# cfpark00/vdm4cdm

Hardware: AMD Instinct MI355X
Metric: 3D voxels/sec UNet fwd+bwd @128^3 (VDM training step) (higher is better)
Workload: dtype bf16; 1 GPU; c3: 128^3 conditional VDM (trainVDM3D128_c_c thick_lowbatch), chs [32, 64, 128, 256], batch 2/GPU, full training step (diffuse + UNet fwd + ELBO + UNet bwd + clip + AdamW), dropout 0.1; global_batch=2, cube=128, parallelism=dp1

## Files before the change

include/vdm4cdm_hip.h:

```cpp
#ifndef VDM4CDM_HIP_H
#define VDM4CDM_HIP_H

#include <stddef.h>
#include <stdint.h>

#ifdef __cplusplus
extern "C" {
#endif

#define VDM_ABI_VERSION 15

typedef enum { VDM_OK = 0, VDM_ERR_ARG = -1, VDM_ERR_HIP = -2, VDM_ERR_UNSUPPORTED = -3 } vdm_status;
typedef enum { VDM_F32 = 0, VDM_BF16 = 1 } vdm_dtype;
typedef enum { VDM_PAD_ZEROS = 0, VDM_PAD_CIRCULAR = 1 } vdm_pad_mode;
typedef enum { VDM_PACK_FWD = 0, VDM_PACK_DGRAD = 1 } vdm_pack_mode;

typedef struct {
    int32_t n, od, oh, ow;
    int32_t cin, cout;
    int32_t ksize;
    int32_t stride;
    int32_t upsample;
    int32_t pad_mode;
    int32_t dtype;
    int32_t out_f32;
} vdm_conv_desc;

const char* vdm_last_error(void);
int vdm_abi_version(void);
int vdm_device_info(int device, int* cu_count, int* lds_bytes, char* arch_name);

size_t vdm_conv_packed_bytes(const vdm_conv_desc* d, int pack_mode);
int vdm_conv_pack_weights(const vdm_conv_desc* d, int pack_mode, const float* w_master, void* w_packed, void* stream);
#define VDM_PACK_CHUNK 16384
typedef struct vdm_pack_item {
    const float* w_master;
    void* w_packed;
    int32_t taps, cout, cin, nc, nchunks, nkb, dgrad, variant, cls_kind, dtype;
    int64_t elems;
} vdm_pack_item;
typedef struct vdm_pack_chunk {
    int32_t item;
    int32_t count;
    int64_t first;
} vdm_pack_chunk;
int vdm_conv_pack_plan(const vdm_conv_desc* d, int pack_mode, const float* w_master, void* w_packed, vdm_pack_item* item);
int vdm_conv_pack_many(const vdm_pack_item* items_device, const vdm_pack_chunk* chunks_device, int nchunks, int dtype, void* stream);
int vdm_conv_gn_tiles(const vdm_conv_desc* d);
int vdm_conv_fwd(const vdm_conv_desc* d, const void* x, const void* w_packed_fwd, const float* bias,
                 const float* nbias, int64_t nbias_stride, const void* residual, void* out, float* gn_partials, void* stream);
int vdm_conv_fwd_gn_supported(const vdm_conv_desc* d);
int vdm_conv_fwd_gn(const vdm_conv_desc* d, const void* x, const void* w_packed_fwd, const float* bias, const float* nbias,
                    int64_t nbias_stride, const void* residual, void* out, float* gn_partials, const float* stats,
                    const float* gamma, const float* beta, int groups, float eps, void* stream);
int vdm_conv_dgrad(const vdm_conv_desc* d, const void* dout, const void* w_packed_dgrad, const void* residual, void* dx,
                   void* stream);
typedef struct vdm_gn_fold {
    const void* x1;
    const void* x2;
    int32_t c1, c2, groups;
    const float* stats;
    const float* gamma;
    const float* beta;
    float eps;
    float inv_keep;
    const uint8_t* keep_mask;
    float* partials;
} vdm_gn_fold;
int vdm_conv_dgrad_gn_tiles(const vdm_conv_desc* d);
int vdm_conv_dgrad_gn(const vdm_conv_desc* d, const void* dout, const void* w_packed_dgrad, void* dyh, const vdm_gn_fold* fold,
                      void* stream);
#define VDM_CONV_VARIANT_GENERIC 0
#define VDM_CONV_VARIANT_CLASS 1
#define VDM_CONV_VARIANT_KPACK 2
#define VDM_CONV_VARIANT_SPLIT 3
#define VDM_CONV_VARIANT_KSPLIT 4
int vdm_conv_kernel_variant(const vdm_conv_desc* d, int dgrad);

int vdm_conv_dgw_supported(const vdm_conv_desc* d);
int vdm_conv_dgw_tiles(const vdm_conv_desc* d);
size_t vdm_conv_dgw_workspace_bytes(const vdm_conv_desc* d);
int vdm_conv_dgrad_gn_wgrad(const vdm_conv_desc* d, const void* dout, const void* w_packed_dgrad, const void* act, void* dyh,
                            const vdm_gn_fold* fold, float* dw, float* dbias, int accumulate, void* workspace, size_t workspace_bytes,
                            void* stream);

size_t vdm_conv_wgrad_workspace_bytes(const vdm_conv_desc* d);
int vdm_conv_wgrad(const vdm_conv_desc* d, const void* x, const void* dout, float* dw, float* dbias, int accumulate,
                   void* workspace, size_t workspace_bytes, void* stream);

#define VDM_WGRAD_THIN_IN 0
#define VDM_WGRAD_THIN_OUT 1
#define VDM_WGRAD_ROWS 2
#define VDM_WGRAD_ROWS_ROLL 3
#define VDM_WGRAD_TAPSPLIT 4
#define VDM_WGRAD_CLASS 5
typedef struct {
    int32_t kernel;
    int32_t tz, ty;
    int32_t workgroups;
    int32_t tiles;
    int32_t P;
    size_t workspace_bytes;
} vdm_wgrad_plan_info;
int vdm_conv_wgrad_plan(const vdm_conv_desc* d, int want_bias, int accumulate, vdm_wgrad_plan_info* out);

#define VDM_GN_STATS_WS_BYTES (2048 * 2 * 64 * 4)
int vdm_gn_stats(const void* x1, int c1, const void* x2, int c2, int n, int64_t voxels, int groups,
                 int dtype, float* stats, float* workspace, const float* part1, int tiles1, const float* part2, int tiles2,
                 float* chsum, void* stream);
int vdm_gn_silu_fwd(const void* x1, int c1, const void* x2, int c2, int n, int64_t voxels, int groups,
                    int dtype, const float* stats, const float* gamma, const float* beta, float eps,
                    float dropout_p, uint64_t seed, void* y, uint8_t* keep_mask, int linear, const int32_t* seed_step, void* stream);
int vdm_gn_dyh(const void* x1, int c1, const void* x2, int c2, int n, int64_t voxels, int groups, int dtype, const float* stats,
               const float* gamma, const float* beta, float eps, float dropout_p, uint64_t seed, const void* dy, void* dyh, int linear,
               const int32_t* seed_step, void* stream);

int vdm_gn_bwd_finalize(const float* partials, int tiles, int n, int c, int groups, int64_t voxels, const float* stats,
                        const float* gamma, float eps, const float* chsum, float* red, float* chan, float* colsum,
                        int64_t colsum_stride, void* stream);
int vdm_gn_bwd_apply(const void* x1, int c1, const void* x2, int c2, int n, int64_t voxels, int groups, int dtype,
                     const float* stats, const float* gamma, float eps, const void* dyh, const float* red, const float* chan,
                     const void* add1, const void* add2, void* dx1, void* dx2, float* dgamma, float* dbeta, void* stream);

int vdm_gn_bwd_apply_wgrad_thin(const void* x, int c, int n, int od, int oh, int ow, int groups, const float* stats, const float* gamma,
                                float eps, const void* dyh, const float* red, const float* chan, const void* add, const void* thin_x,
                                int thin_c, int circular, float* dgamma, float* dbeta, float* dw, float* dbias, void* workspace,
                                size_t workspace_bytes, void* stream);
int vdm_gn_skip_supported(int c1, int c2, int cout, int dtype);
size_t vdm_gn_skip_ws_floats(int c1, int c2, int cout, int n, int64_t voxels);
int vdm_gn_silu_skip_fwd(const void* x1, int c1, const void* x2, int c2, int n, int64_t voxels, int groups, int dtype,
                         const float* stats, const float* gamma, const float* beta, float eps, const float* w1, const float* w2,
                         const float* bias, int cout, void* y, void* skip_out, void* stream);
int vdm_gn_bwd_apply_skip(const void* x1, int c1, const void* x2, int c2, int n, int64_t voxels, int groups, int dtype,
                          const float* stats, const float* gamma, float eps, const void* dyh, const float* red, const float* chan,
                          const void* dout, const float* w1, const float* w2, int cout, void* dx1, void* dx2, float* dgamma,
                          float* dbeta, float* dw1, float* dw2, float* workspace, size_t workspace_floats, void* stream);

int vdm_pack_input(const float* a, const float* b, int64_t nvox, int cpad, int dtype, void* out, void* stream);

typedef struct vdm_cond_mlp {
    const float* input;
    int32_t in_dim, dim, sinusoid, reserved;
    const float* w1; const float* b1;
    const float* w2; const float* b2;
    const float* wproj;
    float* dw1; float* db1; float* dw2; float* db2; float* dwproj;
} vdm_cond_mlp;
size_t vdm_cond_saved_floats(const vdm_cond_mlp* mlps, int n, int rows);
size_t vdm_cond_bwd_scratch_floats(const vdm_cond_mlp* mlps, int n, int rows, int width);
int vdm_cond_table_fwd(const vdm_cond_mlp* mlps, int n, int rows, int width, float* table, float* saved, void* stream);
int vdm_cond_table_bwd(const vdm_cond_mlp* mlps, int n, int rows, int width, const float* dtable, int64_t dtable_stride,
                       const float* saved, float* scratch, float* dbias, void* stream);
int vdm_cond_table_step(const float* table_t, const float* table_v, const int32_t* step_ptr, int rows, int width, float* out,
                        void* stream);
int vdm_cond_input_grad(const vdm_cond_mlp* mlps, int n, int rows, int width, const float* saved, const float* scratch,
                        float* const* host_dinputs, void* stream);

int vdm_diffuse(const float* x, const float* eps, const float* alpha, const float* sigma, int n, int64_t per,
                float* z_t, void* stream);
#define VDM_REDUCE_WS_ROWS 2048
int vdm_loss_terms(const float* x, const float* eps, const float* eps_hat, const float* eps0, float sigma0_over_alpha0,
                   const float* coef, int n, int64_t per, float* sums, float* d_eps_hat, float* workspace, void* stream);

int vdm_diffuse_pack(const float* x, const float* s_cond, const float* eps, uint64_t seed, uint64_t stream_id, const int32_t* seed_step,
                     const float* alpha, const float* sigma, int n, int64_t per, int dtype, float* z_t, void* packed, void* stream);
int vdm_loss_terms_rng(const float* x, const float* eps, uint64_t seed_eps, uint64_t stream_eps, const float* eps_hat, const float* eps0,
                       uint64_t seed_eps0, uint64_t stream_eps0, const int32_t* seed_step, float sigma0_over_alpha0, const float* coef, int n,
                       int64_t per, float* sums, float* d_eps_hat, float* workspace, void* stream);

int vdm_conv_in_dgrad(const void* dh, int n, int d, int h, int w, int c, int dtype, int pad_mode, const float* weight, int cin,
                      float* dz, float* ds, void* stream);
int vdm_schedule_grad_sums(const float* dz, const float* x, const float* eps, uint64_t seed_eps, uint64_t stream_eps,
                           const int32_t* seed_step, int n, int64_t per, float* sums, float* workspace, void* stream);

typedef struct {
    const float* field;
    float* out;
    float alpha, mean, std;
} vdm_augment_channel;
typedef struct {
    int32_t sim;
    int32_t anchor[3];
    int32_t flip[3];
    int32_t perm[3];
} vdm_augment_sample;
int vdm_augment_batch(const vdm_augment_channel* host_channels, int n_channels, int fullsize, int crop,
                      const vdm_augment_sample* host_samples, int n_samples, void* stream);

int vdm_attn_split_heads(const void* src, int64_t src_stride, int64_t src_offset, int n, int64_t voxels, int heads, int head_dim,
                         int dtype, void* rowmajor, void* transposed, void* stream);
int vdm_attn_fwd(const void* q, const void* k, const void* vt, int n, int64_t voxels, int heads, int head_dim, int dtype, float scale,
                 void* out, float* lse, void* stream);
int vdm_attn_rowdot(const void* a, const void* b, int n, int64_t voxels, int heads, int head_dim, int dtype, float* out, void* stream);
int vdm_attn_bwd(const void* q, const void* k, const void* v, const void* qt, const void* kt, const void* do_rowmajor,
                 const void* do_transposed, const float* lse, const float* dsum, int n, int64_t voxels, int heads, int head_dim,
                 int dtype, float scale, void* dqkv, void* stream);
int vdm_channel_sums(const void* x, int64_t rows, int c, int dtype, float* out, void* stream);
int vdm_channel_dot_sums(const void* a, const void* b1, int c1, const void* b2, int c2, int n, int64_t rows_per_sample, int dtype,
                         float* out, void* stream);

int vdm_train_scalars(const float* u0, const float* times, int batch, int rank, int world, float gamma_min, float gamma_max,
                      float bpd_over_batch, float* out, uint64_t seed, const int32_t* seed_step, void* stream);
int vdm_elbo_assemble(const float* sums, const float* coef, int batch, float c_lat0, float c_lat1, float c_rec0, float c_rec1,
                      float* out, void* stream);
int vdm_clip_scale(float* x, int64_t n, const float* sumsq, float max_norm, void* stream);

int vdm_ancestral_step(float* z, const float* eps_hat, const float* noise, const float* coef, const int32_t* step_ptr,
                       uint64_t seed, int64_t n, void* stream);
int vdm_ancestral_step_cfg(float* z, const float* eps_cond, const float* eps_uncond, float w_cfg, const float* noise,
                           const float* coef, const int32_t* step_ptr, uint64_t seed, int64_t n, void* stream);
int vdm_ancestral_step_rows(float* z, const float* eps_hat, const float* eps_uncond, float w_cfg, const float* coef,
                            const int32_t* step_ptr, const uint64_t* seeds, int rows, int64_t per_row, void* stream);
int vdm_randn(float* out, int64_t n, uint64_t seed, uint64_t stream_id, const int32_t* seed_step, void* stream);
int vdm_step_inc(int32_t* step_ptr, void* stream);

typedef struct vdm_ddnm_tables {
    const float* coef;
    const int32_t* sched;
    const int32_t* cursor;
    int32_t n_coef, n_sched;
    const uint64_t* seeds;
    int32_t batch_stream, reserved;
} vdm_ddnm_tables;
int vdm_ddnm_x0(const float* z, const float* eps_hat, const float* eps_uncond, float w_cfg, const vdm_ddnm_tables* tables, float* x0,
                int64_t n, void* stream);
int vdm_ddnm_update(float* z, const float* x0, const float* atax0, const float* aty, int aty_rows, const float* noise,
                    const vdm_ddnm_tables* tables, float* x_r, int rows, int64_t per_row, void* stream);
int vdm_ddnm_mask_step(float* z, const float* eps_hat, const float* eps_uncond, float w_cfg, const float* mask, int mask_rows,
                       const float* y, int y_rows, const float* noise, const vdm_ddnm_tables* tables, float* x_r, int rows,
                       int64_t per_row, void* stream);
int vdm_ddnm_blockmean_step(float* z, const float* eps_hat, const float* eps_uncond, float w_cfg, const float* y, int y_rows, int d, int h,
                            int w, int fz, int fy, int fx, const float* noise, const vdm_ddnm_tables* tables, float* x_r, int rows,
                            void* stream);
int vdm_ddnm_travel(float* z, const float* noise, const vdm_ddnm_tables* tables, const float* travel, int outer, int64_t draw, int rows,
                    int64_t per_row, void* stream);
int vdm_ddnm_advance(int32_t* cursor, const int32_t* sched, int n_sched, int32_t* k_ptr, void* stream);

int vdm_sumsq(const float* x, int64_t n, float* out, float* workspace, void* stream);

#ifdef __cplusplus
}
#endif
#endif
```

vdm4cdm_amd/_lib.py:

```python
import ctypes as C
import os
import subprocess

_HERE = os.path.dirname(os.path.abspath(__file__))
FP32_EXACT = os.environ.get("VDM4CDM_FP32_EXACT", "0") == "1"
LIB_PATH = os.environ.get("VDM4CDM_LIB") or os.path.join(_HERE, "libvdm4cdm_hip_fp32exact.so" if FP32_EXACT else "libvdm4cdm_hip.so")
CSRC = os.path.join(_HERE, "csrc")

VDM_F32, VDM_BF16 = 0, 1
PAD_ZEROS, PAD_CIRCULAR = 0, 1
PACK_FWD, PACK_DGRAD = 0, 1
WGRAD_THIN_IN, WGRAD_THIN_OUT, WGRAD_ROWS, WGRAD_ROWS_ROLL, WGRAD_TAPSPLIT, WGRAD_CLASS = range(6)
GN_STATS_WS_BYTES = 2048 * 2 * 64 * 4


class ConvDesc(C.Structure):
    _fields_ = [(k, C.c_int32) for k in
                ("n", "od", "oh", "ow", "cin", "cout", "ksize", "stride", "upsample", "pad_mode", "dtype", "out_f32")]


class PackItem(C.Structure):
    _fields_ = [("w_master", C.c_void_p), ("w_packed", C.c_void_p)] + \
               [(k, C.c_int32) for k in ("taps", "cout", "cin", "nc", "nchunks", "nkb", "dgrad", "variant", "cls_kind", "dtype")] + \
               [("elems", C.c_int64)]


class PackChunk(C.Structure):
    _fields_ = [("item", C.c_int32), ("count", C.c_int32), ("first", C.c_int64)]


class GnFold(C.Structure):
    _fields_ = [("x1", C.c_void_p), ("x2", C.c_void_p), ("c1", C.c_int32), ("c2", C.c_int32), ("groups", C.c_int32),
                ("stats", C.c_void_p), ("gamma", C.c_void_p), ("beta", C.c_void_p), ("eps", C.c_float), ("inv_keep", C.c_float),
                ("keep_mask", C.c_void_p), ("partials", C.c_void_p)]


class WgradPlanInfo(C.Structure):
    _fields_ = [(k, C.c_int32) for k in ("kernel", "tz", "ty", "workgroups", "tiles", "P")] + [("workspace_bytes", C.c_size_t)]


class CondMlp(C.Structure):
    _fields_ = [("input", C.c_void_p), ("in_dim", C.c_int32), ("dim", C.c_int32), ("sinusoid", C.c_int32), ("reserved", C.c_int32),
                ("w1", C.c_void_p), ("b1", C.c_void_p), ("w2", C.c_void_p), ("b2", C.c_void_p), ("wproj", C.c_void_p),
                ("dw1", C.c_void_p), ("db1", C.c_void_p), ("dw2", C.c_void_p), ("db2", C.c_void_p), ("dwproj", C.c_void_p)]


class AugmentChannel(C.Structure):
    _fields_ = [("field", C.c_void_p), ("out", C.c_void_p), ("alpha", C.c_float), ("mean", C.c_float), ("std", C.c_float)]


class AugmentSample(C.Structure):
    _fields_ = [("sim", C.c_int32), ("anchor", C.c_int32 * 3), ("flip", C.c_int32 * 3), ("perm", C.c_int32 * 3)]


class DdnmTables(C.Structure):
    _fields_ = [("coef", C.c_void_p), ("sched", C.c_void_p), ("cursor", C.c_void_p), ("n_coef", C.c_int32), ("n_sched", C.c_int32),
                ("seeds", C.c_void_p), ("batch_stream", C.c_int32), ("reserved", C.c_int32)]


PACK_CHUNK = 16384
_p, _i, _i64, _u64, _f, _sz = C.c_void_p, C.c_int, C.c_int64, C.c_uint64, C.c_float, C.c_size_t
_D = C.POINTER(ConvDesc)
_T = C.POINTER(DdnmTables)
ABI_VERSION = 15

SIGNATURES = {
    "vdm_last_error": (C.c_char_p, []),
    "vdm_abi_version": (_i, []),
    "vdm_device_info": (_i, [_i, C.POINTER(_i), C.POINTER(_i), C.c_char_p]),
    "vdm_conv_packed_bytes": (_sz, [_D, _i]),
    "vdm_conv_pack_weights": (_i, [_D, _i, _p, _p, _p]),
    "vdm_conv_pack_plan": (_i, [_D, _i, _p, _p, C.POINTER(PackItem)]),
    "vdm_conv_pack_many": (_i, [_p, _p, _i, _i, _p]),
    "vdm_conv_gn_tiles": (_i, [_D]),
    "vdm_conv_fwd": (_i, [_D, _p, _p, _p, _p, _i64, _p, _p, _p, _p]),
    "vdm_conv_fwd_gn_supported": (_i, [_D]),
    "vdm_conv_fwd_gn": (_i, [_D, _p, _p, _p, _p, _i64, _p, _p, _p, _p, _p, _p, _i, _f, _p]),
    "vdm_conv_dgrad": (_i, [_D, _p, _p, _p, _p, _p]),
    "vdm_conv_dgrad_gn_tiles": (_i, [_D]),
    "vdm_conv_dgrad_gn": (_i, [_D, _p, _p, _p, C.POINTER(GnFold), _p]),
    "vdm_conv_kernel_variant": (_i, [_D, _i]),
    "vdm_conv_dgw_supported": (_i, [_D]),
    "vdm_conv_dgw_tiles": (_i, [_D]),
    "vdm_conv_dgw_workspace_bytes": (_sz, [_D]),
    "vdm_conv_dgrad_gn_wgrad": (_i, [_D, _p, _p, _p, _p, C.POINTER(GnFold), _p, _p, _i, _p, _sz, _p]),
    "vdm_conv_wgrad_workspace_bytes": (_sz, [_D]),
    "vdm_conv_wgrad": (_i, [_D, _p, _p, _p, _p, _i, _p, _sz, _p]),
    "vdm_conv_wgrad_plan": (_i, [_D, _i, _i, C.POINTER(WgradPlanInfo)]),
    "vdm_gn_stats": (_i, [_p, _i, _p, _i, _i, _i64, _i, _i, _p, _p, _p, _i, _p, _i, _p, _p]),
    "vdm_gn_silu_fwd": (_i, [_p, _i, _p, _i, _i, _i64, _i, _i, _p, _p, _p, _f, _f, _u64, _p, _p, _i, _p, _p]),
    "vdm_gn_dyh": (_i, [_p, _i, _p, _i, _i, _i64, _i, _i, _p, _p, _p, _f, _f, _u64, _p, _p, _i, _p, _p]),
    "vdm_gn_bwd_finalize": (_i, [_p, _i, _i, _i, _i, _i64, _p, _p, _f, _p, _p, _p, _p, _i64, _p]),
    "vdm_gn_bwd_apply": (_i, [_p, _i, _p, _i, _i, _i64, _i, _i, _p, _p, _f, _p, _p, _p, _p, _p, _p, _p, _p, _p, _p]),
    "vdm_gn_bwd_apply_wgrad_thin": (_i, [_p, _i, _i, _i, _i, _i, _i, _p, _p, _f, _p, _p, _p, _p, _p, _i, _i, _p, _p, _p, _p, _p, _sz, _p]),
    "vdm_gn_skip_supported": (_i, [_i, _i, _i, _i]),
    "vdm_gn_skip_ws_floats": (_sz, [_i, _i, _i, _i, _i64]),
    "vdm_gn_silu_skip_fwd": (_i, [_p, _i, _p, _i, _i, _i64, _i, _i, _p, _p, _p, _f, _p, _p, _p, _i, _p, _p, _p]),
    "vdm_gn_bwd_apply_skip": (_i, [_p, _i, _p, _i, _i, _i64, _i, _i, _p, _p, _f, _p, _p, _p, _p, _p, _p, _i, _p, _p, _p, _p, _p, _p, _p, _sz, _p]),
    "vdm_pack_input": (_i, [_p, _p, _i64, _i, _i, _p, _p]),
    "vdm_cond_saved_floats": (_sz, [C.POINTER(CondMlp), _i, _i]),
    "vdm_cond_bwd_scratch_floats": (_sz, [C.POINTER(CondMlp), _i, _i, _i]),
    "vdm_cond_table_fwd": (_i, [C.POINTER(CondMlp), _i, _i, _i, _p, _p, _p]),
    "vdm_cond_table_bwd": (_i, [C.POINTER(CondMlp), _i, _i, _i, _p, _i64, _p, _p, _p, _p]),
    "vdm_cond_table_step": (_i, [_p, _p, _p, _i, _i, _p, _p]),
    "vdm_cond_input_grad": (_i, [C.POINTER(CondMlp), _i, _i, _i, _p, _p, C.POINTER(_p), _p]),
    "vdm_augment_batch": (_i, [C.POINTER(AugmentChannel), _i, _i, _i, C.POINTER(AugmentSample), _i, _p]),
    "vdm_attn_split_heads": (_i, [_p, _i64, _i64, _i, _i64, _i, _i, _i, _p, _p, _p]),
    "vdm_attn_fwd": (_i, [_p, _p, _p, _i, _i64, _i, _i, _i, _f, _p, _p, _p]),
    "vdm_attn_rowdot": (_i, [_p, _p, _i, _i64, _i, _i, _i, _p, _p]),
    "vdm_attn_bwd": (_i, [_p, _p, _p, _p, _p, _p, _p, _p, _p, _i, _i64, _i, _i, _i, _f, _p, _p]),
    "vdm_channel_sums": (_i, [_p, _i64, _i, _i, _p, _p]),
    "vdm_channel_dot_sums": (_i, [_p, _p, _i, _p, _i, _i, _i64, _i, _p, _p]),
    "vdm_diffuse": (_i, [_p, _p, _p, _p, _i, _i64, _p, _p]),
    "vdm_loss_terms": (_i, [_p, _p, _p, _p, _f, _p, _i, _i64, _p, _p, _p, _p]),
    "vdm_diffuse_pack": (_i, [_p, _p, _p, _u64, _u64, _p, _p, _p, _i, _i64, _i, _p, _p, _p]),
    "vdm_loss_terms_rng": (_i, [_p, _p, _u64, _u64, _p, _p, _u64, _u64, _p, _f, _p, _i, _i64, _p, _p, _p, _p]),
    "vdm_conv_in_dgrad": (_i, [_p, _i, _i, _i, _i, _i, _i, _i, _p, _i, _p, _p, _p]),
    "vdm_schedule_grad_sums": (_i, [_p, _p, _p, _u64, _u64, _p, _i, _i64, _p, _p, _p]),
    "vdm_ancestral_step": (_i, [_p, _p, _p, _p, _p, _u64, _i64, _p]),
    "vdm_ancestral_step_cfg": (_i, [_p, _p, _p, _f, _p, _p, _p, _u64, _i64, _p]),
    "vdm_ancestral_step_rows": (_i, [_p, _p, _p, _f, _p, _p, _p, _i, _i64, _p]),
    "vdm_ddnm_x0": (_i, [_p, _p, _p, _f, _T, _p, _i64, _p]),
    "vdm_ddnm_update": (_i, [_p, _p, _p, _p, _i, _p, _T, _p, _i, _i64, _p]),
    "vdm_ddnm_mask_step": (_i, [_p, _p, _p, _f, _p, _i, _p, _i, _p, _T, _p, _i, _i64, _p]),
    "vdm_ddnm_blockmean_step": (_i, [_p, _p, _p, _f, _p, _i, _i, _i, _i, _i, _i, _i, _p, _T, _p, _i, _p]),
    "vdm_ddnm_travel": (_i, [_p, _p, _T, _p, _i, _i64, _i, _i64, _p]),
    "vdm_ddnm_advance": (_i, [_p, _p, _i, _p, _p]),
    "vdm_randn": (_i, [_p, _i64, _u64, _u64, _p, _p]),
    "vdm_step_inc": (_i, [_p, _p]),
    "vdm_sumsq": (_i, [_p, _i64, _p, _p, _p]),
    "vdm_train_scalars": (_i, [_p, _p, _i, _i, _i, _f, _f, _f, _p, _u64, _p, _p]),
    "vdm_elbo_assemble": (_i, [_p, _p, _i, _f, _f, _f, _f, _p, _p]),
    "vdm_clip_scale": (_i, [_p, _i64, _p, _f, _p]),
}


class VdmError(RuntimeError):
    pass


_lib = None


def build(force=False):
    if force:
        subprocess.check_call(["make", "-C", CSRC, "clean"])
    subprocess.check_call(["make", "-C", CSRC, "-j4"])
    return LIB_PATH


def lib():
    global _lib
    if _lib is not None:
        return _lib
    if not os.path.exists(LIB_PATH):
        raise VdmError(
            f"{LIB_PATH} is missing: the HIP extension is not built. Run `python -c 'import __graft_entry__ as g; g.build()'` "
            "(or `make -C vdm4cdm_amd/csrc`). There is no CPU fallback for the HIP backend.")
    handle = C.CDLL(LIB_PATH)
    for name, (res, args) in SIGNATURES.items():
        fn = getattr(handle, name)
        fn.restype = res
        fn.argtypes = args
    ver = handle.vdm_abi_version()
    if ver != ABI_VERSION:
        raise VdmError(f"libvdm4cdm_hip.so ABI version {ver} != {ABI_VERSION}")
    _lib = handle
    return _lib


def check(status, what=""):
    if status != 0:
        msg = lib().vdm_last_error().decode("utf-8", "replace")
        raise VdmError(f"{what} failed with status {status}: {msg}")
```

vdm4cdm_amd/csrc/conv_api.hip:

```cpp
#include <algorithm>

#include "conv_common.h"

using namespace vdm;

__device__ ClsMasks g_cls_masks[3];

template <typename T>
__device__ __forceinline__ float pack_value(const vdm_pack_item& it, const float* __restrict__ w, size_t r, int lane, int j) {
    constexpr int EPL = DT<T>::EPL, KB = DT<T>::KB;
    const int dgrad = it.dgrad, cout_m = it.cout, cin_m = it.cin, nc = it.nc;
    const int O = dgrad ? cin_m : cout_m, K = dgrad ? cout_m : cin_m;
    const int ct = r % nc; r /= nc;
    const int m = lane & 15, q = lane >> 4;
    if (it.variant == VDM_CONV_VARIANT_KPACK) {
        const int g = r % 7; r /= 7;
        const int chunk = (int)r;
        const int o = chunk * nc * 16 + nc * 4 * (m >> 2) + 4 * ct + (m & 3);
        const int tap = 4 * g + q;
        if (!(o < O && j < K && tap < 27)) return 0.f;
        return dgrad ? w[((size_t)(26 - tap) * cout_m + j) * cin_m + o] : w[((size_t)tap * cout_m + o) * cin_m + j];
    }
    if (it.variant == VDM_CONV_VARIANT_CLASS) {
        const int slot = r % 64; r /= 64;
        const int kb = r % it.nkb; r /= it.nkb;
        const int chunk = (int)r;
        const int o = chunk * nc * 16 + nc * 4 * (m >> 2) + 4 * ct + (m & 3);
        const int k = kb * KB + q * EPL + j;
        float v = 0.f;
        if (o < O && k < K) {
            const unsigned mask = g_cls_masks[it.cls_kind].m[slot];
            for (int t = 0; t < 27; ++t)
                if ((mask >> t) & 1u) v += dgrad ? w[((size_t)t * cout_m + k) * cin_m + o] : w[((size_t)t * cout_m + o) * cin_m + k];
        }
        return v;
    }
    const int taps = it.taps;
    const int tap = r % taps; r /= taps;
    const int kb = r % it.nkb; r /= it.nkb;
    const int chunk = (int)r;
    const int o = chunk * nc * 16 + nc * 4 * (m >> 2) + 4 * ct + (m & 3);
    const int k = kb * KB + q * EPL + j;
    if (!(o < O && k < K)) return 0.f;
    return dgrad ? w[((size_t)(taps - 1 - tap) * cout_m + k) * cin_m + o] : w[((size_t)tap * cout_m + o) * cin_m + k];
}

template <typename T>
__global__ void __launch_bounds__(256) pack_many_kernel(const vdm_pack_item* __restrict__ items, const vdm_pack_chunk* __restrict__ chunks) {
    constexpr int EPL = DT<T>::EPL, FRAG = 64 * EPL;
    const vdm_pack_chunk c = chunks[blockIdx.x];
    const vdm_pack_item it = items[c.item];
    const float* w = it.w_master;
    T* out = reinterpret_cast<T*>(it.w_packed);
    const int j = threadIdx.x % EPL;
    for (long long f = c.first; f < c.first + c.count; f += FRAG) {
        const size_t r = (size_t)(f / FRAG);
#pragma unroll
        for (int u = 0; u < FRAG / 256; ++u) {
            const int e = threadIdx.x + u * 256;
            st_packed_w<T>(out, (size_t)(f + e), pack_value<T>(it, w, r, e / EPL, j));
        }
    }
}

template <typename T>
__global__ void pack_item_kernel(const vdm_pack_item it) {
    constexpr int EPL = DT<T>::EPL;
    for (size_t i = (size_t)blockIdx.x * blockDim.x + threadIdx.x; i < (size_t)it.elems; i += (size_t)gridDim.x * blockDim.x)
        st_packed_w<T>(reinterpret_cast<T*>(it.w_packed), i, pack_value<T>(it, it.w_master, i / (64 * EPL), (int)(i / EPL % 64), (int)(i % EPL)));
}

extern "C" size_t vdm_conv_packed_bytes(const vdm_conv_desc* d, int pack_mode) {
    return validate(d) == VDM_OK ? plan_of(d, pack_mode == VDM_PACK_DGRAD).packed_bytes : 0;
}

extern "C" int vdm_conv_pack_plan(const vdm_conv_desc* d, int pack_mode, const float* w_master, void* w_packed, vdm_pack_item* item) {
    int e = validate(d);
    if (e) return e;
    VDM_REQUIRE(item && w_master && w_packed, "conv_pack_plan: NULL pointer");
    VDM_REQUIRE(pack_mode == VDM_PACK_FWD || pack_mode == VDM_PACK_DGRAD, "conv_pack_plan: bad mode %d", pack_mode);
    const Plan p = plan_of(d, pack_mode == VDM_PACK_DGRAD);
    item->w_master = w_master; item->w_packed = w_packed;
    item->taps = p.taps; item->cout = d->cout; item->cin = d->cin; item->nc = p.nc; item->nchunks = p.nchunks; item->nkb = p.nkb;
    item->dgrad = pack_mode == VDM_PACK_DGRAD;
    item->variant = p.layout; item->cls_kind = p.cls_kind;
    item->dtype = d->dtype;
    item->elems = (long long)(p.packed_bytes / (d->dtype == VDM_F32 ? 4 : 2));
    return VDM_OK;
}

static int upload_cls_masks() {
    static unsigned long long masks_up = 0;
    const int dev = current_device();
    if (dev < 64 && ((masks_up >> dev) & 1ull)) return VDM_OK;
    ClsMasks h[3];
    ClsTable tab;
    for (int k = 0; k < 3; ++k) build_cls(k, tab, h[k]);
    int e = check_hip(hipMemcpyToSymbol(HIP_SYMBOL(g_cls_masks), h, sizeof(h)), "hipMemcpyToSymbol(g_cls_masks)");
    if (!e && dev < 64) masks_up |= 1ull << dev;
    return e;
}

extern "C" int vdm_conv_pack_weights(const vdm_conv_desc* d, int pack_mode, const float* w_master, void* w_packed, void* stream) {
    vdm_pack_item it;
    int e = vdm_conv_pack_plan(d, pack_mode, w_master, w_packed, &it);
    if (!e && it.variant == VDM_CONV_VARIANT_CLASS) e = upload_cls_masks();
    if (e) return e;
    const unsigned grid = (unsigned)((it.elems + 255) / 256 < 2048 ? (it.elems + 255) / 256 : 2048);
    if (d->dtype == VDM_F32)
        hipLaunchKernelGGL(pack_item_kernel<float>, dim3(grid), dim3(256), 0, (hipStream_t)stream, it);
    else
        hipLaunchKernelGGL(pack_item_kernel<bf16_t>, dim3(grid), dim3(256), 0, (hipStream_t)stream, it);
    VDM_LAUNCH_CHECK("pack_item_kernel");
    return VDM_OK;
}

extern "C" int vdm_conv_pack_many(const vdm_pack_item* items_dev, const vdm_pack_chunk* chunks_dev, int nchunks, int dtype, void* stream) {
    VDM_REQUIRE(items_dev && chunks_dev && nchunks > 0, "conv_pack_many: empty work list");
    VDM_REQUIRE(dtype == VDM_F32 || dtype == VDM_BF16, "conv_pack_many: bad dtype %d", dtype);
    int e = upload_cls_masks();
    if (e) return e;
    hipStream_t s = (hipStream_t)stream;
    if (dtype == VDM_F32)
        hipLaunchKernelGGL(pack_many_kernel<float>, dim3(nchunks), dim3(256), 0, s, items_dev, chunks_dev);
    else
        hipLaunchKernelGGL(pack_many_kernel<bf16_t>, dim3(nchunks), dim3(256), 0, s, items_dev, chunks_dev);
    VDM_LAUNCH_CHECK("pack_many_kernel");
    return VDM_OK;
}

static ConvArgs conv_args(const vdm_conv_desc* d, const Plan& p) {
    ConvArgs a{};
    fill_dims(a, d);
    a.Cin = p.K; a.CinStride = cpad(p.K, d->dtype); a.Cout = p.O;
    a.nchunks = p.nchunks; a.nkb = p.nkb;
    return a;
}

extern "C" int vdm_conv_gn_tiles(const vdm_conv_desc* d) {
    return validate(d) == VDM_OK ? plan_of(d, 0).tiles : 0;
}

extern "C" int vdm_conv_fwd(const vdm_conv_desc* d, const void* x, const void* w_packed, const float* bias, const float* nbias,
                            int64_t nbias_stride, const void* residual, void* out, float* gn_partials, void* stream) {
    int e = validate(d);
    if (e) return e;
    VDM_REQUIRE(x && w_packed && out, "conv_fwd: NULL pointer");
    const Plan p = plan_of(d, 0);
    if (p.family == VDM_CONV_VARIANT_CLASS) {
        VDM_REQUIRE(!nbias && !d->out_f32, "conv_fwd: the up-sampling conv takes no per-sample bias / fp32 output");
        return run_cls(d, p, x, w_packed, bias, residual, out, (hipStream_t)stream, gn_partials);
    }
    ConvArgs a = conv_args(d, p);
    a.x = x; a.w = w_packed; a.bias = bias; a.nbias = nbias; a.nbias_stride = nbias_stride; a.res = residual; a.out = out;
    a.gnp = gn_partials;
    return launch_fwd(a, p, (hipStream_t)stream);
}

extern "C" int vdm_conv_fwd_gn_supported(const vdm_conv_desc* d) {
    if (validate(d) != VDM_OK) return 0;
    if (d->dtype != VDM_BF16 || d->ksize != 3 || d->stride != 1 || d->upsample || d->cin > 512 || d->cin % 8) return 0;
    const int family = plan_of(d, 0).family;
    return family == VDM_CONV_VARIANT_GENERIC || family == VDM_CONV_VARIANT_SPLIT;
}

extern "C" int vdm_conv_fwd_gn(const vdm_conv_desc* d, const void* x, const void* w_packed, const float* bias, const float* nbias,
                               int64_t nbias_stride, const void* residual, void* out, float* gn_partials, const float* stats,
                               const float* gamma, const float* beta, int groups, float eps, void* stream) {
    int e = validate(d);
    if (e) return e;
    VDM_REQUIRE(x && w_packed && out && stats && gamma && beta, "conv_fwd_gn: NULL pointer");
    VDM_REQUIRE(vdm_conv_fwd_gn_supported(d), "conv_fwd_gn: this conv has no GroupNorm prologue (vdm_conv_fwd_gn_supported)");
    VDM_REQUIRE(groups > 0 && groups <= 64 && d->cin % groups == 0, "conv_fwd_gn: %d channels / %d groups", d->cin, groups);
    const Plan p = plan_of(d, 0);
    ConvArgs a = conv_args(d, p);
    a.x = x; a.w = w_packed; a.bias = bias; a.nbias = nbias; a.nbias_stride = nbias_stride; a.res = residual; a.out = out;
    a.gnp = gn_partials;
    a.gstats = stats; a.ggamma = gamma; a.gbeta = beta; a.gG = groups; a.geps = eps;
    a.gcnt = (float)((double)d->od * d->oh * d->ow * (d->cin / groups));
    return launch_fwd_gnp(a, p, (hipStream_t)stream);
}

extern "C" int vdm_conv_dgrad(const vdm_conv_desc* d, const void* dout, const void* w_packed_dgrad, const void* residual, void* dx,
                              void* stream) {
    int e = validate(d);
    if (e) return e;
    VDM_REQUIRE(dout && w_packed_dgrad && dx, "conv_dgrad: NULL pointer");
    const Plan p = plan_of(d, 1);
    if (p.family == VDM_CONV_VARIANT_CLASS) return run_cls(d, p, dout, w_packed_dgrad, nullptr, residual, dx, (hipStream_t)stream);
    ConvArgs a = conv_args(d, p);
    a.x = dout; a.w = w_packed_dgrad; a.res = residual; a.out = dx;
    return launch_fwd(a, p, (hipStream_t)stream);
}

extern "C" int vdm_conv_dgrad_gn_tiles(const vdm_conv_desc* d) {
    if (validate(d) != VDM_OK || d->ksize != 3 || d->stride != 1 || d->upsample) return 0;
    return plan_of(d, 1).tiles;
}

extern "C" int vdm_conv_dgrad_gn(const vdm_conv_desc* d, const void* dout, const void* w_packed_dgrad, void* dyh, const vdm_gn_fold* f,
                                 void* stream) {
    int e = validate(d);
    if (e) return e;
    VDM_REQUIRE(dout && w_packed_dgrad && dyh && f, "conv_dgrad_gn: NULL pointer");
    VDM_REQUIRE(d->ksize == 3 && d->stride == 1 && !d->upsample, "conv_dgrad_gn: only the 3x3x3 stride-1 conv feeds a GroupNorm backward");
    VDM_REQUIRE(f->x1 && f->stats && f->gamma && f->beta && f->partials && f->groups > 0, "conv_dgrad_gn: NULL pointer in the fold");
    const int C = d->cin;
    const Plan p = plan_of(d, 1);
    VDM_REQUIRE(f->c1 + f->c2 == C && (f->c2 == 0 || f->x2), "conv_dgrad_gn: c1 + c2 must equal the conv's input channels (%d)", C);
    VDM_REQUIRE(C % f->groups == 0 && C % (p.nc * 4) == 0 && C % epl_of(d->dtype) == 0, "conv_dgrad_gn: channel count %d not supported", C);
    VDM_REQUIRE(f->c2 == 0 || f->c1 % (p.nc * 4) == 0, "conv_dgrad_gn: a lane's %d channels would straddle the concat boundary", p.nc * 4);
    ConvArgs a = conv_args(d, p);
    a.x = dout; a.w = w_packed_dgrad; a.out = dyh; a.gnp = f->partials;
    a.gx1 = f->x1; a.gx2 = f->x2; a.gc1 = f->c1; a.gc2 = f->c2; a.gG = f->groups;
    a.gstats = f->stats; a.ggamma = f->gamma; a.gbeta = f->beta; a.gmask = f->keep_mask;
    a.geps = f->eps; a.ginv_keep = f->keep_mask ? f->inv_keep : 1.0f;
    a.gcnt = (float)((double)d->od * d->oh * d->ow * (C / f->groups));
    return launch_fwd_gnb(a, p, (hipStream_t)stream);
}

extern "C" int vdm_conv_kernel_variant(const vdm_conv_desc* d, int dgrad) {
    return validate(d) ? -1 : plan_of(d, dgrad).family;
}

extern "C" size_t vdm_conv_wgrad_workspace_bytes(const vdm_conv_desc* d) {
    if (validate(d) != VDM_OK) return 0;
    size_t need = 0;
    for (int k = 0; k < 4; ++k) need = std::max(need, plan_wgrad(d, (k & 1) != 0, (k & 2) != 0).workspace_bytes);
    return need;
}

extern "C" int vdm_conv_wgrad_plan(const vdm_conv_desc* d, int want_bias, int accumulate, vdm_wgrad_plan_info* out) {
    int e = validate(d);
    if (e) return e;
    VDM_REQUIRE(out, "conv_wgrad_plan: NULL pointer");
    const WgradPlan p = plan_wgrad(d, want_bias != 0, accumulate != 0);
    out->kernel = p.kernel; out->tz = p.tz; out->ty = p.ty;
    out->workgroups = p.grid; out->tiles = p.ntiles; out->P = p.P;
    out->workspace_bytes = p.workspace_bytes;
    if (want_bias && d->ksize == 1) { set_error("conv_wgrad: fused bias gradient is only built for ksize 3"); return VDM_ERR_UNSUPPORTED; }
    return VDM_OK;
}

extern "C" int vdm_conv_wgrad(const vdm_conv_desc* d, const void* x, const void* dout, float* dw, float* dbias, int accumulate,
                              void* workspace, size_t workspace_bytes, void* stream) {
    int e = validate(d);
    if (e) return e;
    VDM_REQUIRE(x && dout && dw && workspace, "conv_wgrad: NULL pointer");
    const WgradPlan p = plan_wgrad(d, dbias != nullptr, accumulate != 0);
    hipStream_t s = (hipStream_t)stream;
    if (p.kernel == VDM_WGRAD_THIN_IN || p.kernel == VDM_WGRAD_THIN_OUT) {
        const bool in = p.kernel == VDM_WGRAD_THIN_IN;
        ThinArgs a{};
        a.dense = (const bf16_t*)(in ? dout : x);
        a.N = d->n; a.Dz = d->od; a.Dy = d->oh; a.Dx = d->ow; a.C = in ? d->cout : d->cin; a.circular = d->pad_mode == VDM_PAD_CIRCULAR;
        return launch_wgrad_thin(a, false, p, in ? x : dout, d->cin, dw, dbias, workspace, workspace_bytes, s);
    }
    WgradArgs w{};
    fill_dims(w.c, d);
    w.c.x = x;
    w.c.Cin = d->cin; w.c.CinStride = cpad(d->cin, d->dtype); w.c.Cout = d->cout;
    w.dout = dout; w.dout_stride = cpad(d->cout, d->dtype);
    w.slabs = (float*)workspace;
    w.ncb = p.ncb; w.nkb = p.nkb;
    return launch_wgrad_any(w, p, dw, dbias, accumulate, workspace_bytes, d->dtype, s);
}


#ifdef VDM_TIMELINE
namespace vdm { unsigned long long* g_timeline_stamps = nullptr; }
extern "C" int vdm_debug_set_stamps(void* buf) {
    vdm::g_timeline_stamps = (unsigned long long*)buf;
    return VDM_OK;
}
#endif
```

vdm4cdm_amd/csrc/conv_common.h:

```cpp
#pragma once
#include <stdarg.h>
#include <stdio.h>
#include <stdlib.h>
#include <string.h>

#include "common.h"

namespace vdm {

static inline int cdiv(int a, int b) { return (a + b - 1) / b; }
static constexpr int GNP_TABLE_BYTES = 512 * 2 * 4;
static constexpr int GN_SCRATCH_BYTES = 8 * 64 * 2 * 4;

template <int KS_, int STRIDE_, int TZ_, int TY_, int NW_ = 4>
struct Geo {
    static constexpr int KS = KS_, STRIDE = STRIDE_, TZ = TZ_, TY = TY_, TX = 16;
    static constexpr int NW = NW_;
    static constexpr int PAD = KS / 2;
    static constexpr int TAPS = KS * KS * KS;
    static constexpr int HZ = (TZ - 1) * STRIDE + KS, HY = (TY - 1) * STRIDE + KS, HX = (TX - 1) * STRIDE + KS;
    static constexpr int HVOX = HZ * HY * HX;
    static constexpr int ROWS = TZ * TY;
    static constexpr int NV = ROWS / NW;
    static constexpr int OVOX = ROWS * 16;
// ... 665 lines not shown
                for (int c = 0; c < NC; ++c)
                    *reinterpret_cast<float4*>(reinterpret_cast<float*>(out) + vo + c * 4) =
                        make_float4(val[c * 4], val[c * 4 + 1], val[c * 4 + 2], val[c * 4 + 3]);
            } else {
                uint16_t* o16 = reinterpret_cast<uint16_t*>(out) + vo;
                if (NC == 1) {
                    *reinterpret_cast<uint2*>(o16) = make_uint2(pack_bf16x2(val[0], val[1]), pack_bf16x2(val[2], val[3]));
                } else {
#pragma unroll
                    for (int i = 0; i < NC / 2; ++i)
                        *reinterpret_cast<uint4*>(o16 + i * 8) =
                            make_uint4(pack_bf16x2(val[i * 8], val[i * 8 + 1]), pack_bf16x2(val[i * 8 + 2], val[i * 8 + 3]),
                                       pack_bf16x2(val[i * 8 + 4], val[i * 8 + 5]), pack_bf16x2(val[i * 8 + 6], val[i * 8 + 7]));
                }
            }
        } else {
#pragma unroll
            for (int j = 0; j < NC * 4; ++j) {
                if (cbase + j < a.Cout) {
                    float o = val[j];
                    if (res) o += ld_elem<T>(res + vo + j);
                    st_elem<TO>(out + vo + j, o);
                }
            }
        }
    }
    if (a.gnp)
        gn_partials_reduce<NC, G::NW>(gs, gq, gn_sm, a.gnp + ((size_t)n * (a.ntz * a.nty * a.ntx) + tile) * a.Cout * 2, cout0, a.Cout,
                                      cwave, lane, qstride);
}

template <typename T, int SUB>
__device__ __forceinline__ void st_sub(T* p, const float (&f)[SUB]) {
    constexpr int EPL = DT<T>::EPL;
    if constexpr (SUB >= EPL) {
#pragma unroll
        for (int i = 0; i < SUB / EPL; ++i) {
            Piece<T> pc;
#pragma unroll
            for (int j = 0; j < EPL; ++j) pc.f[j] = f[i * EPL + j];
            *reinterpret_cast<uint4*>(p + i * EPL) = pc.store();
        }
    } else {
        *reinterpret_cast<uint2*>(p) = make_uint2(pack_bf16x2(f[0], f[1]), pack_bf16x2(f[2], f[3]));
    }
}

#ifndef VDM_GNB_PACKED
#define VDM_GNB_PACKED 1
#endif
#ifndef VDM_GNB_TABLE
#define VDM_GNB_TABLE 1
#endif
typedef float f32x2 __attribute__((ext_vector_type(2)));
template <typename T, int NC, int NV>
struct GnbRegs {
    static constexpr int EPL = DT<T>::EPL;
    static constexpr int CH = NC * 4;
    static constexpr int SUB = CH >= 8 ? 8 : 4;
    static constexpr int NSUB = CH / SUB;
    static constexpr int XQ = (SUB * (int)sizeof(T) + 15) / 16;
    static constexpr int NBT = CH >= EPL ? CH / EPL : 1;
    uint4 x[NV][NSUB][XQ];
    uint32_t mb[NV];
    float A[CH], B[CH];
};

template <typename T, int NC, int NV>
struct GnbLane {
    const T* xsrc; int xc, xoff, cbase; bool lane_ok;
    __device__ __forceinline__ GnbLane(const ConvArgs& a, int n, int lane, int cout0, int qstride) {
        const int q = lane >> 4;
        const int cbase0 = cout0 + q * qstride;
        lane_ok = cbase0 + NC * 4 <= a.Cout;
        cbase = lane_ok ? cbase0 : 0;
        const bool first = cbase < a.gc1;
        xc = first ? a.gc1 : a.gc2;
        xoff = first ? cbase : cbase - a.gc1;
        xsrc = reinterpret_cast<const T*>(first ? a.gx1 : a.gx2) + (size_t)n * ((size_t)a.Dz * a.Dy * a.Dx * xc);
    }
};

template <typename T, typename G, int NC, int NV>
__device__ __forceinline__ void gnb_issue_row(GnbRegs<T, NC, NV>& r, const GnbLane<T, NC, NV>& L, const RowMap<G, NV>& rm, const ConvArgs& a,
                                              int n, int v) {
    using R = GnbRegs<T, NC, NV>;
    constexpr int EPL = R::EPL, SUB = R::SUB, NSUB = R::NSUB;
    const int PPV = a.Cout / EPL;
    const unsigned vox = rm.ok(a, v) ? rm.vox(a, v) : 0u;
#pragma unroll
    for (int sc = 0; sc < NSUB; ++sc) {
        const T* px = L.xsrc + vox * L.xc + L.xoff + sc * SUB;
        if constexpr (SUB * sizeof(T) >= 16) {
#pragma unroll
            for (int k = 0; k < R::XQ; ++k) r.x[v][sc][k] = reinterpret_cast<const uint4*>(px)[k];
        } else {
            const uint2 u = *reinterpret_cast<const uint2*>(px);
            r.x[v][sc][0] = make_uint4(u.x, u.y, 0u, 0u);
        }
    }
    uint32_t m = 0xffffffffu;
    if (a.gmask) {
        const unsigned char* pm = a.gmask + (size_t)n * ((size_t)a.Dz * a.Dy * a.Dx * PPV) + vox * (unsigned)PPV + L.cbase / EPL;
        m = 0;
#pragma unroll
        for (int k = 0; k < R::NBT; ++k) m |= (uint32_t)pm[k] << (8 * k);
    }
    r.mb[v] = m;
}

template <typename T, int NC, int NV>
__device__ __forceinline__ void gnb_issue_consts(GnbRegs<T, NC, NV>& r, const GnbLane<T, NC, NV>& L, const ConvArgs& a, int n) {
    const int gs = a.Cout / a.gG;
#pragma unroll
    for (int j = 0; j < NC * 4; ++j) {
        const int c = L.cbase + j;
        const int g = c / gs;
        const float sum = a.gstats[((size_t)n * a.gG + g) * 2], sq = a.gstats[((size_t)n * a.gG + g) * 2 + 1];
        const float mean = sum / a.gcnt;
        const float var = fmaxf(sq / a.gcnt - mean * mean, 0.f);
        const float rstd = rsqrtf(var + a.geps);
        const float A = rstd * a.ggamma[c];
        r.A[j] = -1.44269504089f * A;
        r.B[j] = -1.44269504089f * (a.gbeta[c] - mean * A);
    }
}

constexpr int GNB_TABLE_BYTES = 64 * 2 * 4;
__device__ __forceinline__ void gnb_consts_table(float* tab, const ConvArgs& a, int n, int cout0, int tid) {
    if (tid < 64) {
        const int c = cout0 + tid;
        float A2 = 0.f, B2 = 0.f;
        if (c < a.Cout) {
            const int gs = a.Cout / a.gG;
            const int g = c / gs;
            const float sum = a.gstats[((size_t)n * a.gG + g) * 2], sq = a.gstats[((size_t)n * a.gG + g) * 2 + 1];
            const float mean = sum / a.gcnt;
            const float var = fmaxf(sq / a.gcnt - mean * mean, 0.f);
            const float rstd = rsqrtf(var + a.geps);
            const float A = rstd * a.ggamma[c];
            A2 = -1.44269504089f * A;
            B2 = -1.44269504089f * (a.gbeta[c] - mean * A);
        }
        tab[2 * tid] = A2;
        tab[2 * tid + 1] = B2;
    }
}
template <typename T, int NC, int NV>
__device__ __forceinline__ void gnb_consts_read(GnbRegs<T, NC, NV>& r, const float* tab, int lane, int qstride) {
    const float* t = tab + 2 * ((lane >> 4) * qstride);
#pragma unroll
    for (int j = 0; j < NC * 4; j += 2) {
        const float4 v = *reinterpret_cast<const float4*>(t + 2 * j);
        r.A[j] = v.x; r.B[j] = v.y; r.A[j + 1] = v.z; r.B[j + 1] = v.w;
    }
}

template <typename T, typename G, int NC, int NV, bool TABLED = false>
__device__ __forceinline__ void gnb_issue(GnbRegs<T, NC, NV>& r, const ConvArgs& a, int n, int oz0, int oy0, int ox0, int cwave, int lane,
                                          int cout0, int qstride) {
    const GnbLane<T, NC, NV> L(a, n, lane, cout0, qstride);
    const RowMap<G, NV> rm(a, oz0, oy0, ox0, cwave, lane);
#pragma unroll
    for (int v = 0; v < NV; ++v) gnb_issue_row<T, G, NC, NV>(r, L, rm, a, n, v);
    if constexpr (!TABLED) gnb_issue_consts<T, NC, NV>(r, L, a, n);
}

template <typename T, int SUB, int XQ>
__device__ __forceinline__ void raw_unpack(const uint4 (&q)[XQ], float (&f)[SUB]) {
    if constexpr (sizeof(T) == 4) {
#pragma unroll
        for (int k = 0; k < XQ; ++k) {
            f[4 * k] = __builtin_bit_cast(float, q[k].x); f[4 * k + 1] = __builtin_bit_cast(float, q[k].y);
            f[4 * k + 2] = __builtin_bit_cast(float, q[k].z); f[4 * k + 3] = __builtin_bit_cast(float, q[k].w);
        }
    } else {
        const uint32_t w[4] = {q[0].x, q[0].y, q[0].z, q[0].w};
#pragma unroll
        for (int i = 0; i < SUB / 2; ++i) {
            f[2 * i] = __builtin_bit_cast(float, w[i] << 16);
            f[2 * i + 1] = __builtin_bit_cast(float, w[i] & 0xffff0000u);
        }
    }
}

template <typename T, typename G, int NC, int NV, bool PREFETCHED, bool TABLED = false>
__device__ __forceinline__ void conv_epilogue_gnb(const f32x4 (&acc)[NV][NC], const ConvArgs& a, GnbRegs<T, NC, NV>& r, int n,
                                                  int oz0, int oy0, int ox0, int cwave, int lane, float* gn_sm, int tile, int cout0,
                                                  int qstride, const float* ctab = nullptr) {
    using R = GnbRegs<T, NC, NV>;
    constexpr int EPL = R::EPL, CH = R::CH, SUB = R::SUB, NSUB = R::NSUB;
    constexpr int PD = NV < 3 ? NV : 3;
    const int q = lane >> 4;
    const int cbase = cout0 + q * qstride;
    const int C = a.Cout;
    const GnbLane<T, NC, NV> L(a, n, lane, cout0, qstride);
    const RowMap<G, NV> rm(a, oz0, oy0, ox0, cwave, lane);
    if constexpr (!PREFETCHED) {
#pragma unroll
        for (int v = 0; v < PD; ++v) gnb_issue_row<T, G, NC, NV>(r, L, rm, a, n, v);
        if constexpr (!TABLED) gnb_issue_consts<T, NC, NV>(r, L, a, n);
    }
    if constexpr (TABLED) gnb_consts_read<T, NC, NV>(r, ctab, lane, qstride);
    float gsum[CH], gsq[CH];
#pragma unroll
    for (int j = 0; j < CH; ++j) gsum[j] = gsq[j] = 0.f;
    f32x2 gs2[CH / 2], gq2[CH / 2];
#pragma unroll
    for (int j = 0; j < CH / 2; ++j) gs2[j] = gq2[j] = f32x2{0.f, 0.f};
    const bool lane_ok = cbase + CH <= C;
    T* out = reinterpret_cast<T*>(a.out) + (size_t)n * ((size_t)a.Dz * a.Dy * a.Dx * C);
#pragma unroll
    for (int v = 0; v < NV; ++v) {
        if constexpr (!PREFETCHED) {
            if (v + PD < NV) gnb_issue_row<T, G, NC, NV>(r, L, rm, a, n, v + PD);
        }
        if (!rm.ok(a, v) || !lane_ok) continue;
        const unsigned vox = rm.vox(a, v);
        const uint32_t mb = r.mb[v];
        if constexpr (sizeof(T) == 2 && VDM_GNB_PACKED) {
            const uint32_t ikb = __builtin_bit_cast(uint32_t, a.ginv_keep);
            const uint32_t mbs = CH >= EPL ? mb : (mb >> ((unsigned)cbase % EPL));
#pragma unroll
            for (int sc = 0; sc < NSUB; ++sc) {
                const uint32_t w[4] = {r.x[v][sc][0].x, r.x[v][sc][0].y, r.x[v][sc][0].z, r.x[v][sc][0].w};
                uint32_t ow[SUB / 2];
#pragma unroll
                for (int i = 0; i < SUB / 2; ++i) {
                    const int jj = sc * SUB + 2 * i;
                    const f32x2 xv = {__builtin_bit_cast(float, w[i] << 16), __builtin_bit_cast(float, w[i] & 0xffff0000u)};
                    const f32x2 A2 = {r.A[jj], r.A[jj + 1]}, B2 = {r.B[jj], r.B[jj + 1]};
                    const f32x2 yl = xv * A2 + B2;
                    const f32x2 e1 = f32x2{__builtin_amdgcn_exp2f(yl.x), __builtin_amdgcn_exp2f(yl.y)} + 1.0f;
                    const f32x2 sg = {__builtin_amdgcn_rcpf(e1.x), __builtin_amdgcn_rcpf(e1.y)};
                    const f32x2 ds = sg * ((yl * -0.69314718056f) * (1.0f - sg) + 1.0f);
                    const int bit = CH >= EPL ? (jj / EPL) * 8 + jj % EPL : jj;
                    const f32x2 keep = {__builtin_bit_cast(float, (uint32_t)__builtin_amdgcn_sbfe((int)mbs, bit, 1) & ikb),
                                        __builtin_bit_cast(float, (uint32_t)__builtin_amdgcn_sbfe((int)mbs, bit + 1, 1) & ikb)};
                    const f32x2 ac = {acc[v][jj >> 2][jj & 3], acc[v][jj >> 2][(jj & 3) + 1]};
                    const f32x2 dd = ac * (ds * keep);
                    gs2[jj / 2] += dd;
                    gq2[jj / 2] = dd * xv + gq2[jj / 2];
                    ow[i] = pack_bf16x2(dd.x, dd.y);
                }
                T* po = out + (vox * (unsigned)C + (unsigned)(cbase + sc * SUB));
                if constexpr (SUB == 8) *reinterpret_cast<uint4*>(po) = make_uint4(ow[0], ow[1], ow[2], ow[3]);
                else *reinterpret_cast<uint2*>(po) = make_uint2(ow[0], ow[1]);
            }
            continue;
        }
#pragma unroll
        for (int sc = 0; sc < NSUB; ++sc) {
            float xv[SUB], d[SUB];
            raw_unpack<T, SUB, R::XQ>(r.x[v][sc], xv);
#pragma unroll
            for (int j = 0; j < SUB; ++j) {
                const int jj = sc * SUB + j;
                const float yl = fmaf(xv[j], r.A[jj], r.B[jj]);
                const float sg = __builtin_amdgcn_rcpf(1.0f + __builtin_amdgcn_exp2f(yl));
                const float ds = sg * fmaf(-0.69314718056f * yl, 1.0f - sg, 1.0f);
                const int bit = CH >= EPL ? (jj / EPL) * 8 + jj % EPL : (cbase + jj) % EPL;
                const float keep = ((mb >> bit) & 1u) ? a.ginv_keep : 0.f;
                const float dd = acc[v][jj >> 2][jj & 3] * (ds * keep);
                d[j] = dd;
                gsum[jj] += dd;
                gsq[jj] = fmaf(dd, xv[j], gsq[jj]);
            }
            st_sub<T, SUB>(out + (vox * (unsigned)C + (unsigned)(cbase + sc * SUB)), d);
        }
    }
    if constexpr (sizeof(T) == 2 && VDM_GNB_PACKED) {
#pragma unroll
        for (int j = 0; j < CH / 2; ++j) {
            gsum[2 * j] = gs2[j].x; gsum[2 * j + 1] = gs2[j].y;
            gsq[2 * j] = gq2[j].x; gsq[2 * j + 1] = gq2[j].y;
        }
    }
    gn_partials_reduce<NC, G::NW>(gsum, gsq, gn_sm, a.gnp + ((size_t)n * (a.ntz * a.nty * a.ntx) + tile) * a.Cout * 2, cout0, a.Cout, cwave,
                                  lane, qstride);
}

struct ClsEntry { int lds_off; int dx; };
struct ClsTable {
    int n[8];
    ClsEntry e[8][8];
};
struct ClsArgs {
    ConvArgs c;
    ClsTable t;
    int oDz, oDy, oDx;
    int sDz, sDy, sDx;
};
struct ClsMasks { unsigned m[64]; };

struct WgradArgs {
    ConvArgs c;
    const void* dout;
    int dout_stride;
    float* slabs;
    float* bslabs;
    int P;
    int ntiles;
    int ncb, nkb;
};

template <typename T> struct WG;
template <> struct WG<bf16_t> { static constexpr int NT = 2; };
template <> struct WG<float> { static constexpr int NT = 1; };

template <typename T, typename G>
__device__ __forceinline__ void stage_dout_dma_gen(char* lds, const T* __restrict__ g, const ConvArgs& a, int n, int oz0, int oy0,
                                                   int ox0, int cb, int cstride, int sub, int pz, int py, int px, int wave, int lane) {
    constexpr int EPL = DT<T>::EPL, KB = DT<T>::KB, SH = DT<T>::SHIFT;
    const int k = lane >> 2, j = lane & 3;
    const int pc = j ^ ((k >> 1) & 3);
    const int co = cb * KB + pc * EPL;
    const int ox = ox0 + k;
    const int m = sub ? 2 : 1;
    const bool okx = co < a.Cout && ox < a.Dx;
    const unsigned xoff = (__umul24((unsigned)(m * ox + px) & 0xffffffu, (unsigned)cstride) + (unsigned)co) << SH;
    const char* gn = reinterpret_cast<const char*>(g) + (((size_t)n * (m * a.Dz) * (m * a.Dy) * (m * a.Dx) * cstride) << SH);
    const char* zp = reinterpret_cast<const char*>(g_zero_page);
    for (int r = wave; r < G::ROWS; r += 4) {
        const int oz = oz0 + r / G::TY, oy = oy0 + r % G::TY;
        const bool okrow = oz < a.Dz && oy < a.Dy;
        const unsigned fz = okrow ? (unsigned)(m * oz + pz) : 0u, fy = okrow ? (unsigned)(m * oy + py) : 0u;
        const size_t rowel = (size_t)((fz * (unsigned)(m * a.Dy) + fy) * (unsigned)(m * a.Dx)) * (unsigned)cstride;
        const char* src = (okrow && okx) ? gn + (rowel << SH) + xoff : zp;
        __builtin_amdgcn_global_load_lds((const __attribute__((address_space(1))) void*)src,
                                         (__attribute__((address_space(3))) void*)(lds + r * 1024), 16, 0, 0);
    }
}

template <typename T, typename G>
struct DoutRowStager {
    static constexpr int EPL = DT<T>::EPL, KB = DT<T>::KB, SH = DT<T>::SHIFT;
    unsigned xoff;
    bool okx;
    const char* gn;
    int cstride;
    __device__ __forceinline__ DoutRowStager(const T* __restrict__ g, const ConvArgs& a, int n, int ox0, int cb, int cstride_, int lane) : cstride(cstride_) {
        const int k = lane >> 2, j = lane & 3;
        const int pc = j ^ ((k >> 1) & 3);
        const int co = cb * KB + pc * EPL;
        const int ox = ox0 + k;
        okx = co < a.Cout && ox < a.Dx;
        xoff = (__umul24((unsigned)ox & 0xffffffu, (unsigned)cstride) + (unsigned)co) << SH;
        gn = reinterpret_cast<const char*>(g) + (((size_t)n * a.Dz * a.Dy * a.Dx * cstride) << SH);
    }
    __device__ __forceinline__ void row(char* lds, const ConvArgs& a, int oz0, int oy0, int r) const {
        const int oz = oz0 + r / G::TY, oy = oy0 + r % G::TY;
        const bool okrow = oz < a.Dz && oy < a.Dy;
        const unsigned fz = okrow ? (unsigned)oz : 0u, fy = okrow ? (unsigned)oy : 0u;
        const size_t rowel = (size_t)((fz * (unsigned)a.Dy + fy) * (unsigned)a.Dx) * (unsigned)cstride;
        const char* src = (okrow && okx) ? gn + (rowel << SH) + xoff : reinterpret_cast<const char*>(g_zero_page);
        __builtin_amdgcn_global_load_lds((const __attribute__((address_space(1))) void*)src,
                                         (__attribute__((address_space(3))) void*)(lds + r * 1024), 16, 0, 0);
    }
};

template <typename T, typename G>
__device__ __forceinline__ void stage_dout_dma(char* lds, const T* __restrict__ g, const ConvArgs& a, int n, int oz0, int oy0,
                                               int ox0, int cb, int cstride, int wave, int lane) {
    stage_dout_dma_gen<T, G>(lds, g, a, n, oz0, oy0, ox0, cb, cstride, 0, 0, 0, 0, wave, lane);
}

template <typename T, typename G>
__device__ __forceinline__ void stage_dout_dma_sub(char* lds, const T* __restrict__ g, const ConvArgs& a, int n, int oz0, int oy0,
                                                   int ox0, int cb, int cstride, int pz, int py, int px, int wave, int lane) {
    stage_dout_dma_gen<T, G>(lds, g, a, n, oz0, oy0, ox0, cb, cstride, 1, pz, py, px, wave, lane);
}

template <typename T> struct TrFetch;
template <> struct TrFetch<bf16_t> {
    static constexpr int NOFF = 1;
    static __device__ __forceinline__ void lane_off(int (&o)[1], int ct, int xs, int dx, int lane) {
        const int g = lane >> 4, li = lane & 15, qp = li >> 2, p = li & 3;
        const int hx = (4 * g + qp) * xs + dx;
        const int slot = (2 * ct + (p >> 1)) ^ ((hx >> 1) & 3);
        o[0] = hx * 64 + slot * 16 + (p & 1) * 8;
    }
    template <int HI>
    static __device__ __forceinline__ uint4 get(const char* lds, const int (&o)[1], int uni) {
        typedef __attribute__((address_space(3))) s16x4* lptr;
        const char* p = lds + uni + o[0];
        const s16x4 lo = __builtin_amdgcn_ds_read_tr16_b64_v4i16((lptr)(p));
        const s16x4 hi = __builtin_amdgcn_ds_read_tr16_b64_v4i16((lptr)(p + HI));
        const uint2 l2 = __builtin_bit_cast(uint2, lo), h2 = __builtin_bit_cast(uint2, hi);
        return make_uint4(l2.x, l2.y, h2.x, h2.y);
    }
};
template <> struct TrFetch<float> {
    static constexpr int NOFF = 4;
    static __device__ __forceinline__ void lane_off(int (&o)[4], int ct, int xs, int dx, int lane) {
        (void)ct;
        const int m = lane & 15, kq = lane >> 4;
#pragma unroll
        for (int st = 0; st < 4; ++st) {
            const int hx = (4 * st + kq) * xs + dx;
            o[st] = hx * 64 + (((m >> 2) ^ ((hx >> 1) & 3)) * 16) + (m & 3) * 4;
        }
    }
    template <int HI>
    static __device__ __forceinline__ uint4 get(const char* lds, const int (&o)[4], int uni) {
        const char* p = lds + uni;
        uint4 r;
        r.x = *reinterpret_cast<const uint32_t*>(p + o[0]);
        r.y = *reinterpret_cast<const uint32_t*>(p + o[1]);
        r.z = *reinterpret_cast<const uint32_t*>(p + o[2]);
        r.w = *reinterpret_cast<const uint32_t*>(p + o[3]);
        return r;
    }
};


static int nc_for(int cout, int dtype) { return cout <= 16 ? 1 : ((cout <= 32 || dtype == VDM_F32) ? 2 : 4); }
static int epl_of(int dtype) { return dtype == VDM_F32 ? 4 : 8; }
static int kb_of(int dtype) { return dtype == VDM_F32 ? 16 : 32; }
static int cpad(int c, int dtype) { const int e = epl_of(dtype); return (c + e - 1) / e * e; }

static int validate(const vdm_conv_desc* d) {
    VDM_REQUIRE(d != nullptr, "conv desc is NULL");
    VDM_REQUIRE(d->n > 0 && d->od > 0 && d->oh > 0 && d->ow > 0, "conv: bad output dims %d %d %d %d", d->n, d->od, d->oh, d->ow);
    VDM_REQUIRE(d->cin > 0 && d->cout > 0, "conv: bad channels cin=%d cout=%d", d->cin, d->cout);
    VDM_REQUIRE(d->ksize == 1 || d->ksize == 3, "conv: ksize must be 1 or 3 (got %d)", d->ksize);
    VDM_REQUIRE(d->stride == 1 || d->stride == 2, "conv: stride must be 1 or 2 (got %d)", d->stride);
    VDM_REQUIRE(!(d->stride == 2 && d->ksize != 3), "conv: stride 2 needs ksize 3");
    VDM_REQUIRE(!(d->upsample && (d->stride != 1 || d->ksize != 3)), "conv: upsample needs stride 1, ksize 3");
    VDM_REQUIRE(!(d->upsample && ((d->od | d->oh | d->ow) & 1)), "conv: upsample needs even output dims");
    VDM_REQUIRE(d->dtype == VDM_F32 || d->dtype == VDM_BF16, "conv: bad dtype %d", d->dtype);
    VDM_REQUIRE(d->pad_mode == VDM_PAD_ZEROS || d->pad_mode == VDM_PAD_CIRCULAR, "conv: bad pad_mode %d", d->pad_mode);
    VDM_REQUIRE((long long)(d->od > d->oh ? (d->od > d->ow ? d->od : d->ow) : (d->oh > d->ow ? d->oh : d->ow)) * d->stride < (1 << 12),
                "conv: spatial extent too large");
    VDM_REQUIRE(d->cin <= (1 << 16) && d->cout <= (1 << 16) && d->n <= (1 << 20), "conv: channel count / batch out of range");
    const long long fine = (long long)d->od * d->oh * d->ow * (d->stride == 2 ? 8 : 1);
    const long long cmax = cpad(d->cin > d->cout ? d->cin : d->cout, d->dtype);
    VDM_REQUIRE(fine * cmax < (1LL << 32), "conv: %lld voxels x %lld channels per sample exceed the 32-bit in-sample index", fine, cmax);
    return VDM_OK;
}

struct Plan {
    int taps, nc, nchunks, nkb, O, K;
    int dtype, ks, stride, ups, out_f32;
    int N, Dz, Dy, Dx;
    int layout, cls_kind;
    int family;
    int roll, wg8;
    int tz, ty;
    int tiles;
    size_t packed_bytes;
};

static int cu_count();

static int current_device() {
    int dev = 0;
    if (hipGetDevice(&dev) != hipSuccess || dev < 0) dev = 0;
    return dev;
}

template <typename K>
static int set_lds(K kernel, size_t bytes, unsigned long long& done_mask) {
    const int dev = current_device();
    if (dev < 64 && ((done_mask >> dev) & 1ull)) return VDM_OK;
    int e = check_hip(hipFuncSetAttribute(reinterpret_cast<const void*>(kernel), hipFuncAttributeMaxDynamicSharedMemorySize, (int)bytes),
                      "hipFuncSetAttribute(MaxDynamicSharedMemorySize)");
    if (e) return e;
    if (dev < 64) done_mask |= 1ull << dev;
    return VDM_OK;
}

static int cu_count() {
    static int cached[64] = {0};
    const int dev = current_device();
    int n = dev < 64 ? cached[dev] : 0;
    if (n == 0) {
        if (hipDeviceGetAttribute(&n, hipDeviceAttributeMultiprocessorCount, dev) != hipSuccess || n <= 0) n = 256;
        if (dev < 64) cached[dev] = n;
    }
    return n;
}

static void small_grid_tile(Plan& p) {
    const long long per_sample = (long long)p.nchunks * p.N * cdiv(p.Dx, 16);
    const long long tiles48 = per_sample * cdiv(p.Dz, 4) * cdiv(p.Dy, 8), tiles28 = per_sample * cdiv(p.Dz, 2) * cdiv(p.Dy, 8);
    p.tz = 4; p.ty = 8;
    if (const char* f = getenv("VDM4CDM_FORCE_TZ")) {
        p.tz = atoi(f);
        if (p.tz == 1 || p.tz == 2 || p.tz == 4) return;
        p.tz = 4;
    }
    if (tiles48 >= 2LL * cu_count()) return;
    p.tz = 2;
    if (tiles28 >= cu_count()) return;
    p.tz = 1;
    if (2 * tiles28 < cu_count()) p.ty = 4;
}

static bool uses_split(const Plan& p) {
    const long long wgs = (long long)p.nchunks * p.N * cdiv(p.Dz, p.tz) * cdiv(p.Dy, p.ty) * cdiv(p.Dx, 16);
    return p.tz <= 2 && wgs < 2LL * cu_count() && p.O % 64 == 0 && getenv("VDM4CDM_NO_SPLIT") == nullptr;
}

static bool ksplit_tile(Plan& p) {
    static const int level = getenv("VDM4CDM_KSPLIT") ? atoi(getenv("VDM4CDM_KSPLIT")) : 1;
    if (level <= 0 || p.nkb < 4 || p.O % 64 != 0 || p.tz > 2 || (p.tz == 2 && level < 2)) return false;
    if (p.tz == 2) { p.tz = 1; p.ty = 8; }
    return true;
}

static int s2_tile_z() {
    static const int v = getenv("VDM4CDM_S2_TZ") ? atoi(getenv("VDM4CDM_S2_TZ")) : 2;
    return v == 1 ? 1 : 2;
}

enum ClsKind { CLS_UP_FWD = 0, CLS_UP_DGRAD = 1, CLS_S2_DGRAD = 2 };

static int cls_dim_entries(int kind, int p, int o[2], unsigned tapset[2]) {
    if (kind == CLS_S2_DGRAD) {
        if (p == 0) { o[0] = 0; tapset[0] = 1u << 1; return 1; }
        o[0] = +1; tapset[0] = 1u << 0; o[1] = 0; tapset[1] = 1u << 2; return 2;
    }
    if (p == 0) { o[0] = -1; tapset[0] = 1u << 0; o[1] = 0; tapset[1] = (1u << 1) | (1u << 2); return 2; }
    o[0] = 0; tapset[0] = (1u << 0) | (1u << 1); o[1] = +1; tapset[1] = 1u << 2; return 2;
}

static void build_cls(int kind, ClsTable& tab, ClsMasks& masks) {
    using G = Geo<3, 1, 4, 8>;
    for (int i = 0; i < 64; ++i) masks.m[i] = 0;
    for (int cl = 0; cl < 8; ++cl) {
        const int p[3] = {(cl >> 2) & 1, (cl >> 1) & 1, cl & 1};
        int o[3][2];
        unsigned ts[3][2];
        int cnt[3];
        for (int d = 0; d < 3; ++d) cnt[d] = cls_dim_entries(kind, p[d], o[d], ts[d]);
        int ne = 0;
        for (int iz = 0; iz < cnt[0]; ++iz)
            for (int iy = 0; iy < cnt[1]; ++iy)
                for (int ix = 0; ix < cnt[2]; ++ix) {
                    const int hz = kind == CLS_UP_DGRAD ? 1 - o[0][iz] : o[0][iz] + 1;
                    const int hy = kind == CLS_UP_DGRAD ? 1 - o[1][iy] : o[1][iy] + 1;
                    const int hx = kind == CLS_UP_DGRAD ? 1 - o[2][ix] : o[2][ix] + 1;
                    tab.e[cl][ne].lds_off = (hz * G::HY + hy) * G::HX * 64;
                    tab.e[cl][ne].dx = hx;
                    unsigned m = 0;
                    for (int tz = 0; tz < 3; ++tz)
                        for (int ty = 0; ty < 3; ++ty)
                            for (int tx = 0; tx < 3; ++tx)
                                if (((ts[0][iz] >> tz) & 1) && ((ts[1][iy] >> ty) & 1) && ((ts[2][ix] >> tx) & 1)) m |= 1u << ((tz * 3 + ty) * 3 + tx);
                    masks.m[cl * 8 + ne] = m;
                    ++ne;
                }
        tab.n[cl] = ne;
        for (int i = ne; i < 8; ++i) tab.e[cl][i] = tab.e[cl][0];
    }
}

static Plan plan_of(const vdm_conv_desc* d, int dgrad) {
    Plan p{};
    p.taps = d->ksize * d->ksize * d->ksize;
    p.O = dgrad ? d->cin : d->cout;
    p.K = dgrad ? d->cout : d->cin;
    p.nc = nc_for(p.O, d->dtype);
    p.nchunks = cdiv(p.O, p.nc * 16);
    p.nkb = cdiv(p.K, kb_of(d->dtype));
    p.dtype = d->dtype; p.ks = d->ksize;
    p.stride = dgrad ? 1 : d->stride; p.ups = dgrad ? 0 : d->upsample; p.out_f32 = dgrad ? 0 : d->out_f32;
    p.N = d->n; p.Dz = d->od; p.Dy = d->oh; p.Dx = d->ow;
    p.layout = p.family = VDM_CONV_VARIANT_GENERIC;
    p.tz = 4; p.ty = 8;
    size_t slots = (size_t)p.nkb * p.taps;
    const bool bf16io = d->dtype == VDM_BF16 && !p.out_f32;
    if (d->ksize == 3 && (d->upsample || (dgrad && d->stride == 2))) {
        p.layout = p.family = VDM_CONV_VARIANT_CLASS;
        p.cls_kind = d->upsample ? (dgrad ? CLS_UP_DGRAD : CLS_UP_FWD) : CLS_S2_DGRAD;
        if (d->upsample) { p.Dz /= 2; p.Dy /= 2; p.Dx /= 2; }
        slots = (size_t)p.nkb * 64;
    } else if (bf16io && p.ks == 3 && p.stride == 1 && p.K <= 8 && p.O <= 32 && getenv("VDM4CDM_NO_KPACK") == nullptr) {
        p.layout = p.family = VDM_CONV_VARIANT_KPACK;
        slots = 7;
    } else if (p.stride == 2) {
        p.tz = s2_tile_z(); p.ty = 4;
    } else if (p.ks == 3) {
        small_grid_tile(p);
        if (bf16io && p.nc == 4) {
            if (ksplit_tile(p)) p.family = VDM_CONV_VARIANT_KSPLIT;
            else if (uses_split(p)) p.family = VDM_CONV_VARIANT_SPLIT;
        }
        if (bf16io && p.nc == 2 && p.tz == 4) {
            static const bool roll_on = getenv("VDM4CDM_ROLL") ? atoi(getenv("VDM4CDM_ROLL")) != 0 : true;
            static const int wg8_mask = getenv("VDM4CDM_WG8") ? atoi(getenv("VDM4CDM_WG8")) : 0;
            p.roll = p.nkb == 1 && cdiv(p.Dz, 4) >= 4 && roll_on;
            p.wg8 = p.roll ? 0 : (wg8_mask & 3);
        }
    }
    p.tiles = cdiv(p.Dz, p.tz) * cdiv(p.Dy, p.ty) * cdiv(p.Dx, 16) * (p.cls_kind == CLS_UP_FWD && p.family == VDM_CONV_VARIANT_CLASS ? 8 : 1);
    p.packed_bytes = (size_t)p.nchunks * slots * p.nc * 64 * 16;
    return p;
}

static void fill_dims(ConvArgs& a, const vdm_conv_desc* d) {
    a.N = d->n; a.Dz = d->od; a.Dy = d->oh; a.Dx = d->ow;
    a.Iz = d->od * d->stride; a.Iy = d->oh * d->stride; a.Ix = d->ow * d->stride;
    a.Sz = d->upsample ? a.Iz / 2 : a.Iz; a.Sy = d->upsample ? a.Iy / 2 : a.Iy; a.Sx = d->upsample ? a.Ix / 2 : a.Ix;
    a.circular = d->pad_mode == VDM_PAD_CIRCULAR;
}

struct ThinArgs {
    const bf16_t* dense;
    const uint32_t* thin;
    int N, Dz, Dy, Dx, C, circular;
    float* slabs;
    const bf16_t* gx; const bf16_t* gdyh; const bf16_t* gadd;
    const float* gstats; const float* ggamma; const float* gred; const float* gchan;
    float* gdgamma; float* gdbeta;
    int gG; float geps;
    FastDiv fdx, fdy, fdz;
};
constexpr int THIN_COLS = 80;

struct WgradPlan {
    int kernel;
    int ks, stride, tz, ty, nta, ntb;
    int CL, ncb, nkb, npairs;
    int ntz, nty, ntx, ntiles;
    int nseg, zsteps;
    int P;
    int per_wg, grouped;
    int grid;
    size_t slab_bytes;
    size_t workspace_bytes;
};

static int env_int(const char* name, int dflt) { const char* e = getenv(name); return e ? atoi(e) : dflt; }
static int wgrad_wgs() { static const int v = env_int("VDM4CDM_WGRAD_WGS", 512); return v > 0 ? v : 512; }
static int wgrad_thin_wgs() { static const int v = env_int("VDM4CDM_THIN_WGS", 512); return v > 0 ? v : 512; }
static bool wgrad_thin_enabled() { static const bool on = getenv("VDM4CDM_NO_THIN_WGRAD") == nullptr; return on; }
static bool wgrad_rows_enabled() { static const bool on = env_int("VDM4CDM_WGRAD_ROWS", 1) != 0; return on; }
static bool wgrad_roll_enabled() { static const bool on = env_int("VDM4CDM_WGRAD_ROLL", 1) != 0; return on; }
static int wgrad_s2_tile_z() { static const int v = env_int("VDM4CDM_S2W_TZ", 1); return v == 1 ? 1 : 2; }
static bool wgrad_grouped_only() { static const bool on = getenv("VDM4CDM_GROUPED_REDUCE") != nullptr; return on; }

static WgradPlan plan_wgrad_thin(int kernel, int n, int od, int oh, int ow, int cdense) {
    WgradPlan p{};
    p.kernel = kernel; p.ks = 3; p.stride = 1;
    long long want = ((long long)n * od * oh * cdiv(ow, 32) + 3) / 4;
    if (want > wgrad_thin_wgs()) want = wgrad_thin_wgs();
    p.grid = p.P = (int)(want < 1 ? 1 : want);
    p.slab_bytes = (size_t)p.grid * cdense * THIN_COLS * sizeof(float);
    p.workspace_bytes = p.slab_bytes + (size_t)n * od * oh * ow * sizeof(uint32_t);
    return p;
}

static WgradPlan plan_wgrad(const vdm_conv_desc* d, bool want_bias, bool accumulate) {
    const bool bf16 = d->dtype == VDM_BF16, k3s1 = d->ksize == 3 && d->stride == 1 && !d->upsample;
    if (bf16 && k3s1 && !accumulate && wgrad_thin_enabled() && !(d->pad_mode == VDM_PAD_CIRCULAR && d->ow < 17)) {
        const auto dense_ok = [](int c) { return c == 16 || c == 32 || c == 64; };
        if (d->cin <= 2 && dense_ok(d->cout)) return plan_wgrad_thin(VDM_WGRAD_THIN_IN, d->n, d->od, d->oh, d->ow, d->cout);
        if (d->cout == 1 && !want_bias && dense_ok(d->cin)) return plan_wgrad_thin(VDM_WGRAD_THIN_OUT, d->n, d->od, d->oh, d->ow, d->cin);
    }
    WgradPlan p{};
    p.kernel = VDM_WGRAD_TAPSPLIT;
    p.ks = d->ksize; p.stride = d->stride;
    p.CL = bf16 ? 32 : 16;
    p.nta = p.ntb = p.CL / 16;
    p.ncb = cdiv(d->cout, p.CL); p.nkb = cdiv(d->cin, p.CL);
    p.npairs = p.ncb * p.nkb;
    p.per_wg = 1;
    int Dz = d->od, Dy = d->oh, Dx = d->ow, slots = 27, bias_rows = 1;
    if (d->ksize == 1) {
        p.tz = 4; p.ty = 8; p.per_wg = 4; slots = 4;
    } else if (d->stride == 2) {
        p.tz = wgrad_s2_tile_z(); p.ty = 4;
    } else if (d->upsample) {
        p.kernel = VDM_WGRAD_CLASS;
        p.tz = 2; p.ty = 8;
        Dz /= 2; Dy /= 2; Dx /= 2;
        p.npairs *= 8; slots = 8; bias_rows = 8;
    } else {
        p.tz = 2; p.ty = 8;
        if (bf16 && d->cin <= 16) p.ntb = 1;
        else if (bf16 && d->cout <= 16) p.nta = 1;
        else if (bf16 && wgrad_rows_enabled()) p.kernel = VDM_WGRAD_ROWS;
    }
    p.ntz = cdiv(Dz, p.tz); p.nty = cdiv(Dy, p.ty); p.ntx = cdiv(Dx, 16);
    const long long ntiles = (long long)d->n * p.ntz * p.nty * p.ntx;
    p.ntiles = (int)(ntiles < 0x7fffffffLL ? ntiles : 0x7fffffffLL);
    p.P = wgrad_wgs() / p.npairs;
    if (p.P < 1) p.P = 1;
    if (p.P > p.ntiles) p.P = p.ntiles;
    if (p.kernel == VDM_WGRAD_ROWS && wgrad_roll_enabled()) {
        const long long ncols = (long long)d->n * p.nty * p.ntx;
        int nseg = (int)(p.P / ncols);
        if (nseg > p.ntz / 2) nseg = p.ntz / 2;
        if (nseg >= 1 || p.ntz >= 4) {
            if (nseg < 1) nseg = 1;
            p.kernel = VDM_WGRAD_ROWS_ROLL;
            p.zsteps = cdiv(p.ntz, nseg);
            p.nseg = cdiv(p.ntz, p.zsteps);
            p.ntiles = (int)(ncols * p.nseg);
            if (p.P > p.ntiles) p.P = p.ntiles;
        }
    }
    p.grid = p.npairs * p.P;
    p.grouped = p.P * p.per_wg > 32 || wgrad_grouped_only();
    p.slab_bytes = (size_t)p.npairs * p.P * slots * p.CL * p.CL * sizeof(float);
    p.workspace_bytes = p.slab_bytes + (size_t)p.ncb * bias_rows * p.P * p.CL * sizeof(float);
    return p;
}

int launch_fwd(const ConvArgs& a, const Plan& p, hipStream_t s);
int launch_fwd_gnb(const ConvArgs& a, const Plan& p, hipStream_t s);
int launch_fwd_gnp(const ConvArgs& a, const Plan& p, hipStream_t s);
int run_cls(const vdm_conv_desc* d, const Plan& p, const void* x, const void* w, const float* bias, const void* res, void* out,
            hipStream_t s, float* gn_partials = nullptr);
int launch_dgw_reduce(const float* slabs, const float* bslabs, float* dw, float* dbias, int P, int accumulate, hipStream_t s);
int launch_wgrad_any(const WgradArgs& w, const WgradPlan& p, float* dw, float* dbias, int accumulate, size_t workspace_bytes, int dtype,
                     hipStream_t s);
int launch_wgrad_thin(ThinArgs a, bool gna, const WgradPlan& p, const void* thin_src, int cin, float* dw, float* dbias, void* workspace,
                      size_t workspace_bytes, hipStream_t s);

}
```

vdm4cdm_amd/csrc/conv_wgrad.hip:

```cpp
#include "conv_common.h"

namespace vdm {

#ifdef VDM_TIMELINE
#define WG_TL_DECL unsigned long long tl_acc[6] = {0, 0, 0, 0, 0, 0}, tl_last = __builtin_amdgcn_s_memrealtime(); const unsigned long long tl_first = tl_last
#define WG_TL(k)                                                          \
    do {                                                                  \
        __builtin_amdgcn_sched_barrier(0);                                \
        const unsigned long long now_ = __builtin_amdgcn_s_memrealtime(); \
        tl_acc[k] += now_ - tl_last;                                      \
        tl_last = now_;                                                   \
        __builtin_amdgcn_sched_barrier(0);                                \
    } while (0)
#define WG_TL_WRITE(a_)                                                                                     \
    do {                                                                                                    \
        if ((a_).stamps && lane == 0) {                                                                     \
            unsigned long long* o_ = (a_).stamps + ((size_t)blockIdx.x * 4 + wave) * 8;                      \
            for (int k_ = 0; k_ < 6; ++k_) o_[k_] = tl_acc[k_];                                             \
            o_[6] = tl_first;                                                                               \
            o_[7] = __builtin_amdgcn_s_memrealtime();                                                       \
        }                                                                                                   \
    } while (0)
#else
#define WG_TL_DECL do { } while (0)
#define WG_TL(k) do { } while (0)
#define WG_TL_WRITE(a_) do { } while (0)
#endif


template <typename T, int KS, int STRIDE, int UPS, int TZ, int TY, int NTA = WG<T>::NT, int NTB = WG<T>::NT>
__global__ void __launch_bounds__(256, 2) conv_wgrad_kernel(const WgradArgs w) {
    using G = Geo<KS, STRIDE, TZ, TY>;
    using TF = TrFetch<T>;
    constexpr int NT = WG<T>::NT, NOFF = TF::NOFF;
    constexpr bool CLS = (UPS == 2);
    constexpr int TAPS = CLS ? 8 : G::TAPS;
    constexpr int TPW = (TAPS + 3) / 4;
    constexpr int RSTEP = (sizeof(T) == 2) ? 2 : 1;
    constexpr int IN_BYTES = ((G::HVOX + 15) / 16) * 1024;
    static_assert(sizeof(T) == 4 || (TY % 2) == 0, "bf16 k-step = two rows of the same z-slab");
    constexpr int HI_IN = STRIDE * G::HX * 64;
    constexpr int HI_DO = 16 * 64;
    extern __shared__ __attribute__((aligned(16))) char lds[];
    char* lds_in = lds;
    char* lds_do = lds + IN_BYTES;
    const ConvArgs& a = w.c;

    const int tid = threadIdx.x;
    const int lane = tid & 63;
    const int wave = __builtin_amdgcn_readfirstlane(tid >> 6);

    const int pair = blockIdx.x / w.P, pidx = blockIdx.x % w.P;
    const int cls = CLS ? pair / (w.ncb * w.nkb) : 0;
    const int pr = CLS ? pair % (w.ncb * w.nkb) : pair;
    const int cb = pr / w.nkb, kb = pr % w.nkb;
    const int pz = (cls >> 2) & 1, py = (cls >> 1) & 1, px = cls & 1;

    f32x4 acc[TPW][NTA][NTB];
#pragma unroll
    for (int t = 0; t < TPW; ++t)
#pragma unroll
        for (int i = 0; i < NTA; ++i)
#pragma unroll
            for (int j = 0; j < NTB; ++j) acc[t][i][j] = f32x4{0.f, 0.f, 0.f, 0.f};

    int tap_u[TPW];
    int lo_in[TPW][NTB][NOFF];
    int lo_do[NTA][NOFF];
#pragma unroll
    for (int t = 0; t < TPW; ++t) {
        int tap = (TAPS > 1) ? wave + 4 * t : 0;
        if (tap >= TAPS) tap = TAPS - 1;
        const int dz = CLS ? ((tap >> 2) & 1) + pz : tap / (KS * KS), dy = CLS ? ((tap >> 1) & 1) + py : (tap / KS) % KS,
                  dx = CLS ? (tap & 1) + px : tap % KS;
        tap_u[t] = (dz * G::HY + dy) * G::HX * 64;
#pragma unroll
        for (int j = 0; j < NTB; ++j) TF::lane_off(lo_in[t][j], j, STRIDE, dx, lane);
    }
#pragma unroll
    for (int i = 0; i < NTA; ++i) TF::lane_off(lo_do[i], i, 1, 0, lane);
    const int row0 = (TAPS > 1) ? 0 : wave * RSTEP;
    const int rowinc = (TAPS > 1) ? RSTEP : 4 * RSTEP;

    const T* x = reinterpret_cast<const T*>(a.x);
    const T* g = reinterpret_cast<const T*>(w.dout);
    float bsum[DT<T>::EPL];
#pragma unroll
    for (int j = 0; j < DT<T>::EPL; ++j) bsum[j] = 0.f;
    auto in_base = [&](int r) { return (((r / TY) * STRIDE * G::HY + (r % TY) * STRIDE) * G::HX) * 64; };
    WG_TL_DECL;

    for (int tile = pidx; tile < w.ntiles; tile += w.P) {
        int tx, ty, tz, n, rest_;
        decode_tile(a, (uint32_t)tile, tx, ty, tz, n, rest_);
        const int oz0 = tz * TZ, oy0 = ty * TY, ox0 = tx * 16;
        __syncthreads();
        WG_TL(0);
        stage_halo_dma<T, G, CLS ? 0 : UPS>(lds_in, x, a, n, oz0, oy0, ox0, kb, wave, lane);
        if constexpr (CLS)
            stage_dout_dma_sub<T, G>(lds_do, g, a, n, oz0, oy0, ox0, cb, w.dout_stride, pz, py, px, wave, lane);
        else
            stage_dout_dma<T, G>(lds_do, g, a, n, oz0, oy0, ox0, cb, w.dout_stride, wave, lane);
        WG_TL(1);
        __syncthreads();
        WG_TL(2);
        uint4 af[NTA], afn[NTA], bfA[NTB], bfB[NTB];
#pragma unroll
        for (int i = 0; i < NTA; ++i) af[i] = TF::template get<HI_DO>(lds_do, lo_do[i], row0 * 1024);
#pragma unroll
        for (int j = 0; j < NTB; ++j) bfA[j] = TF::template get<HI_IN>(lds_in, lo_in[0][j], in_base(row0) + tap_u[0]);
        for (int r = row0; r < G::ROWS; r += rowinc) {
            const int rn = (r + rowinc < G::ROWS) ? r + rowinc : r;
            const int i0 = in_base(r), in0 = in_base(rn);
#pragma unroll
            for (int t = 0; t < TPW; ++t) {
                uint4 (&cur)[NTB] = (t & 1) ? bfB : bfA;
                uint4 (&nxt)[NTB] = (t & 1) ? bfA : bfB;
                if (t + 1 < TPW) {
#pragma unroll
                    for (int j = 0; j < NTB; ++j) nxt[j] = TF::template get<HI_IN>(lds_in, lo_in[t + 1 < TPW ? t + 1 : 0][j], i0 + tap_u[t + 1 < TPW ? t + 1 : 0]);
                } else {
#pragma unroll
                    for (int i = 0; i < NTA; ++i) afn[i] = TF::template get<HI_DO>(lds_do, lo_do[i], rn * 1024);
#pragma unroll
                    for (int j = 0; j < NTB; ++j) nxt[j] = TF::template get<HI_IN>(lds_in, lo_in[0][j], in0 + tap_u[0]);
                }
                __builtin_amdgcn_sched_barrier(0);
#pragma unroll
                for (int i = 0; i < NTA; ++i)
#pragma unroll
                    for (int j = 0; j < NTB; ++j) mma16_act<T>(acc[t][i][j], af[i], cur[j]);
                __builtin_amdgcn_sched_barrier(0);
            }
#pragma unroll
            for (int i = 0; i < NTA; ++i) af[i] = afn[i];
            if (TPW & 1) {
#pragma unroll
                for (int j = 0; j < NTB; ++j) bfA[j] = bfB[j];
            }
        }
        WG_TL(3);
        if (TAPS > 1 && w.bslabs != nullptr && kb == 0) {
            const int vx = lane >> 2, sl = lane & 3;
#pragma unroll
            for (int r = wave; r < G::ROWS; r += 4) {
                Piece<T> pz;
                pz.load(*reinterpret_cast<const uint4*>(lds_do + r * 1024 + vx * 64 + sl * 16));
#pragma unroll
                for (int j = 0; j < DT<T>::EPL; ++j) bsum[j] += pz.f[j];
            }
        }
        WG_TL(4);
    }

    constexpr int CL = NT * 16;
    if (TAPS > 1 && w.bslabs != nullptr && kb == 0) {
        float* shb = reinterpret_cast<float*>(lds);
        constexpr int EPLc = DT<T>::EPL;
        __syncthreads();
#pragma unroll
        for (int j = 0; j < EPLc; ++j) shb[tid * EPLc + j] = bsum[j];
        __syncthreads();
        if (tid < CL) {
            const int piece = tid / EPLc, j = tid % EPLc;
            float tot = 0.f;
            for (int wv = 0; wv < 4; ++wv)
                for (int vx = 0; vx < 16; ++vx) {
                    const int ln = vx * 4 + (piece ^ ((vx >> 1) & 3));
                    tot += shb[(wv * 64 + ln) * EPLc + j];
                }
            w.bslabs[((size_t)cb * (CLS ? 8 : 1) * w.P + cls * w.P + pidx) * CL + tid] = tot;
        }
    }
    constexpr int SLAB = TAPS * CL * CL;
    const int nslab_per_wg = (TAPS > 1) ? 1 : 4;
    float* slab = w.slabs + ((size_t)(pair * w.P + pidx) * nslab_per_wg + ((TAPS > 1) ? 0 : wave)) * SLAB;
    const int gq = lane >> 4, col = lane & 15;
#pragma unroll
    for (int t = 0; t < TPW; ++t) {
        const int tap = (TAPS > 1) ? wave + 4 * t : 0;
        if (tap >= TAPS) continue;
#pragma unroll
        for (int i = 0; i < NT; ++i)
#pragma unroll
            for (int j = 0; j < NT; ++j)
#pragma unroll
                for (int rg = 0; rg < 4; ++rg)
                    slab[(tap * CL + i * 16 + gq * 4 + rg) * CL + j * 16 + col] = (i < NTA && j < NTB) ? acc[t][i < NTA ? i : 0][j < NTB ? j : 0][rg] : 0.f;
    }
    WG_TL(5);
    WG_TL_WRITE(a);
}

template <int V> struct IntC { static constexpr int value = V; };
template <typename T, int TZ, int TY, int PAR>
__device__ __forceinline__ void wgrad_rows_step(f32x4 (&acc)[27], f32x4& accb, bool bias, const char* lds_in, const char* lds_do,
                                                const int (&lo_a)[1], const int (&lo_b)[3][1]) {
    using G = Geo<3, 1, TZ, TY>;
    using TF = TrFetch<T>;
    constexpr int NJ = TY / 2, NP = NJ + 1, NG = G::HZ * 3, R = G::HZ, ROWB = G::HX * 64;
    auto pair_of = [&](int grp, int p) {
        const int hz = grp / 3, dx = grp % 3;
        return TF::template get<ROWB>(lds_in, lo_b[dx], (((TZ * PAR + hz) % R) * G::HY + 2 * p) * ROWB);
    };
    int lo_w[3][1];
#pragma unroll
    for (int dx = 0; dx < 3; ++dx) {
        lo_w[dx][0] = lo_b[dx][0];
        asm volatile("" : "+v"(lo_w[dx][0]));
    }
    auto wrap_of = [&](int grp) {
        const int hz = grp / 3, dx = grp % 3;
        return TF::template get<(TY - 1) * ROWB>(lds_in, lo_w[dx], (((TZ * PAR + hz) % R) * G::HY + 1) * ROWB);
    };
    uint4 ae[TZ][NJ], ao[TZ][NJ - 1], aw[TZ];
#pragma unroll
    for (int oz = 0; oz < TZ; ++oz) {
#pragma unroll
        for (int j = 0; j < NJ; ++j) ae[oz][j] = TF::template get<1024>(lds_do, lo_a, (oz * TY + 2 * j) * 1024);
#pragma unroll
        for (int m = 0; m < NJ - 1; ++m) ao[oz][m] = TF::template get<1024>(lds_do, lo_a, (oz * TY + 2 * m + 1) * 1024);
        aw[oz] = TF::template get<(TY - 1) * 1024>(lds_do, lo_a, oz * TY * 1024);
    }
    uint4 bp[NP], bw;
#pragma unroll
    for (int p = 0; p < NP; ++p) bp[p] = pair_of(0, p);
    bw = wrap_of(0);
    if (bias) {
        const uint4 ones = make_uint4(0x3f803f80u, 0x3f803f80u, 0x3f803f80u, 0x3f803f80u);
#pragma unroll
        for (int oz = 0; oz < TZ; ++oz)
#pragma unroll
            for (int j = 0; j < NJ; ++j) mma16_act<T>(accb, ae[oz][j], ones);
    }
#pragma unroll
    for (int grp = 0; grp < NG; ++grp) {
        const int hz = grp / 3, dx = grp % 3;
#pragma unroll
        for (int p = 0; p <= NP; ++p) {
            __builtin_amdgcn_sched_barrier(0);
#pragma unroll
            for (int dz = 0; dz < 3; ++dz) {
                const int oz = hz - dz;
                if (oz < 0 || oz >= TZ) continue;
                const int t = dz * 9 + dx;
                if (p == NP) {
                    mma16_act<T>(acc[t + 3], aw[oz], bw);
                } else {
                    if (p < NJ) mma16_act<T>(acc[t], ae[oz][p], bp[p]);
                    if (p >= 1 && p <= NJ - 1) mma16_act<T>(acc[t + 3], ao[oz][p - 1], bp[p]);
                    if (p >= 1) mma16_act<T>(acc[t + 6], ae[oz][p - 1], bp[p]);
                }
            }
            __builtin_amdgcn_sched_barrier(0);
            if (grp + 1 < NG) {
                if (p == NP) bw = wrap_of(grp + 1);
                else bp[p] = pair_of(grp + 1, p);
            }
        }
    }
}

template <typename T, int TZ, int TY, bool ROLL>
__global__ void __launch_bounds__(256, 2) conv_wgrad_rows_kernel(const WgradArgs w) {
    using G = Geo<3, 1, TZ, TY>;
    using TF = TrFetch<T>;
    static_assert(sizeof(T) == 2 && (TY % 2) == 0, "bf16 only: a fragment = two rows of the same z-slab");
    static_assert(!ROLL || TZ == 2, "the ring mapping has period two for TZ = 2");
    constexpr int IN_BYTES = ((G::HVOX + 15) / 16) * 1024;
    constexpr int CL = 32, R = G::HZ;
    extern __shared__ __attribute__((aligned(16))) char lds[];
    char* lds_in = lds;
    char* lds_do = lds + IN_BYTES;
    const ConvArgs& a = w.c;

    const int tid = threadIdx.x;
    const int lane = tid & 63;
    const int wave = __builtin_amdgcn_readfirstlane(tid >> 6);
    const int ia = wave >> 1, jb = wave & 1;
    const int pair = blockIdx.x / w.P, pidx = blockIdx.x % w.P;
    const int cb = pair / w.nkb, kb = pair % w.nkb;

    f32x4 acc[27];
#pragma unroll
    for (int t = 0; t < 27; ++t) acc[t] = f32x4{0.f, 0.f, 0.f, 0.f};
    int lo_a[1], lo_b[3][1];
    TF::lane_off(lo_a, ia, 1, 0, lane);
#pragma unroll
    for (int dx = 0; dx < 3; ++dx) TF::lane_off(lo_b[dx], jb, 1, dx, lane);

    const T* x = reinterpret_cast<const T*>(a.x);
    const T* g = reinterpret_cast<const T*>(w.dout);
    f32x4 accb = f32x4{0.f, 0.f, 0.f, 0.f};
    const bool bias = w.bslabs != nullptr && kb == 0 && jb == 0;
    WG_TL_DECL;
    if constexpr (ROLL) {
        for (int cs = pidx; cs < w.ntiles; cs += w.P) {
            uint32_t b = (uint32_t)cs;
            uint32_t q = fdiv(b, a.fdx);
            const int tx = (int)(b - q * (uint32_t)a.ntx); b = q;
            q = fdiv(b, a.fdy);
            const int ty = (int)(b - q * (uint32_t)a.nty); b = q;
            q = fdiv(b, a.fdz);
            const int seg = (int)(b - q * (uint32_t)a.nseg);
            const int n = (int)q;
            const int zs0 = seg * a.zsteps, zs1 = min(a.ntz, zs0 + a.zsteps);
            const int oy0 = ty * TY, ox0 = tx * 16;
            const RowStager<T, G, 0> st(x, a, n, 0, oy0, ox0, kb, lane, 1, 0, 0, 0, a.Sz, a.Sy, a.Sx);
            auto step = [&](int s, auto parc) {
                const int rel = s - zs0;
                const int p0 = rel == 0 ? 0 : TZ * rel + (R - TZ), cnt = rel == 0 ? R : TZ;
                __syncthreads();
                WG_TL(0);
                for (int r = wave; r < cnt * G::HY; r += 4) {
                    const int sl = r / G::HY, hy = r % G::HY, p = p0 + sl;
                    st.row(lds_in + ((p % R) * G::HY + hy) * (G::HX * 64), a, TZ * zs0 + p, hy);
                }
                stage_dout_dma<T, G>(lds_do, g, a, n, s * TZ, oy0, ox0, cb, w.dout_stride, wave, lane);
                WG_TL(1);
                __syncthreads();
                WG_TL(2);
                wgrad_rows_step<T, TZ, TY, decltype(parc)::value>(acc, accb, bias, lds_in, lds_do, lo_a, lo_b);
                WG_TL(3);
            };
            for (int s = zs0; s < zs1; s += 2) {
                step(s, IntC<0>());
                if (s + 1 < zs1) step(s + 1, IntC<1>());
            }
        }
    } else {
        for (int tile = pidx; tile < w.ntiles; tile += w.P) {
            int tx, ty, tz, n, rest_;
            decode_tile(a, (uint32_t)tile, tx, ty, tz, n, rest_);
            const int oz0 = tz * TZ, oy0 = ty * TY, ox0 = tx * 16;
            __syncthreads();
            WG_TL(0);
            stage_halo_dma<T, G, 0>(lds_in, x, a, n, oz0, oy0, ox0, kb, wave, lane);
            stage_dout_dma<T, G>(lds_do, g, a, n, oz0, oy0, ox0, cb, w.dout_stride, wave, lane);
            WG_TL(1);
            __syncthreads();
            WG_TL(2);
            wgrad_rows_step<T, TZ, TY, 0>(acc, accb, bias, lds_in, lds_do, lo_a, lo_b);
            WG_TL(3);
        }
    }

    if (bias && (lane & 15) == 0) {
#pragma unroll
        for (int rg = 0; rg < 4; ++rg) w.bslabs[((size_t)cb * w.P + pidx) * CL + ia * 16 + (lane >> 4) * 4 + rg] = accb[rg];
    }
    float* slab = w.slabs + (size_t)(pair * w.P + pidx) * (27 * CL * CL);
    const int gq = lane >> 4, col = lane & 15;
#pragma unroll
    for (int t = 0; t < 27; ++t)
#pragma unroll
        for (int rg = 0; rg < 4; ++rg) slab[(t * CL + ia * 16 + gq * 4 + rg) * CL + jb * 16 + col] = acc[t][rg];
    WG_TL(5);
    WG_TL_WRITE(a);
}

constexpr int WRED_OUT = 64, WRED_GRP = 4;
__global__ void __launch_bounds__(256) wgrad_reduce_kernel(const float* __restrict__ slabs, float* __restrict__ dw, int taps,
                                                          int cout, int cin, int ncb, int nkb, int CL, int nslabs, int accumulate) {
    const int total = taps * cout * cin;
    const int o = threadIdx.x % WRED_OUT, sg = threadIdx.x / WRED_OUT;
    const int i = blockIdx.x * WRED_OUT + o;
    __shared__ float part[WRED_GRP][WRED_OUT];
    float sum = 0.f;
    if (i < total) {
        const int ci = i % cin, co = (i / cin) % cout, tap = i / (cin * cout);
        const int pair = (co / CL) * nkb + ci / CL;
        const size_t slab_elems = (size_t)taps * CL * CL;
        const float* s = slabs + (size_t)pair * nslabs * slab_elems + ((size_t)tap * CL + co % CL) * CL + ci % CL;
        int k = sg;
        for (; k + 7 * WRED_GRP < nslabs; k += 8 * WRED_GRP) {
            float v[8];
#pragma unroll
            for (int u = 0; u < 8; ++u) v[u] = s[(size_t)(k + WRED_GRP * u) * slab_elems];
#pragma unroll
            for (int u = 0; u < 8; ++u) sum += v[u];
        }
        for (; k < nslabs; k += WRED_GRP) sum += s[(size_t)k * slab_elems];
    }
    part[sg][o] = sum;
    __syncthreads();
    if (sg == 0 && i < total) {
        float tot = 0.f;
#pragma unroll
        for (int g = 0; g < WRED_GRP; ++g) tot += part[g][o];
        dw[i] = accumulate ? dw[i] + tot : tot;
    }
}
__global__ void __launch_bounds__(256) wgrad_reduce_direct_kernel(const float* __restrict__ slabs, float* __restrict__ dw, int taps,
                                                                 int cout, int cin, int ncb, int nkb, int CL, int nslabs, int accumulate) {
    const int total = taps * cout * cin;
    const int i = blockIdx.x * 256 + threadIdx.x;
    if (i >= total) return;
    const int ci = i % cin, co = (i / cin) % cout, tap = i / (cin * cout);
    const int pair = (co / CL) * nkb + ci / CL;
    const size_t slab_elems = (size_t)taps * CL * CL;
    const float* s = slabs + (size_t)pair * nslabs * slab_elems + ((size_t)tap * CL + co % CL) * CL + ci % CL;
    float sum = 0.f;
    int k = 0;
    for (; k + 7 < nslabs; k += 8) {
        float v[8];
#pragma unroll
        for (int u = 0; u < 8; ++u) v[u] = s[(size_t)(k + u) * slab_elems];
#pragma unroll
        for (int u = 0; u < 8; ++u) sum += v[u];
    }
    for (; k < nslabs; ++k) sum += s[(size_t)k * slab_elems];
    dw[i] = accumulate ? dw[i] + sum : sum;
}
__global__ void __launch_bounds__(256) wgrad_bias_reduce_kernel(const float* __restrict__ bslabs, float* __restrict__ dbias, int cout,
                                                               int CL, int P, int accumulate) {
    const int c = threadIdx.x & 15, gp = threadIdx.x >> 4;
    const int co = blockIdx.x * 16 + c;
    __shared__ float part[16][17];
    float sum = 0.f;
    if (co < cout) {
        const float* s = bslabs + (size_t)(co / CL) * P * CL + co % CL;
        for (int p = gp; p < P; p += 16) sum += s[(size_t)p * CL];
    }
    part[gp][c] = sum;
    __syncthreads();
    if (gp == 0 && co < cout) {
        float tot = 0.f;
#pragma unroll
        for (int k = 0; k < 16; ++k) tot += part[k][c];
        dbias[co] = accumulate ? dbias[co] + tot : tot;
    }
}

__global__ void __launch_bounds__(256) wgrad_cls_reduce_kernel(const float* __restrict__ slabs, float* __restrict__ dw, int cout, int cin,
                                                              int ncb, int nkb, int CL, int P, int accumulate) {
    const int total = 27 * cout * cin;
    const int o = threadIdx.x & 63, sg = threadIdx.x >> 6;
    const int i = blockIdx.x * 64 + o;
    __shared__ float part[4][64];
    float sum = 0.f;
    if (i < total) {
        const int ci = i % cin, co = (i / cin) % cout, tap = i / (cin * cout);
        const int tz = tap / 9, ty = (tap / 3) % 3, tx = tap % 3;
        const size_t slab_elems = (size_t)8 * CL * CL;
        for (int b = 0; b < 8; ++b) {
            const int bz = (b >> 2) & 1, by = (b >> 1) & 1, bx = b & 1;
            const int cls = b, e = (((tz + 1 - bz) >> 1) << 2) | (((ty + 1 - by) >> 1) << 1) | ((tx + 1 - bx) >> 1);
            const int pair = (cls * ncb + co / CL) * nkb + ci / CL;
            const float* s = slabs + (size_t)pair * P * slab_elems + ((size_t)e * CL + co % CL) * CL + ci % CL;
            for (int k = sg; k < P; k += 4) sum += s[(size_t)k * slab_elems];
        }
    }
    part[sg][o] = sum;
    __syncthreads();
    if (sg == 0 && i < total) {
        const float tot = (part[0][o] + part[1][o]) + (part[2][o] + part[3][o]);
        dw[i] = accumulate ? dw[i] + tot : tot;
    }
}

static bool ablate_reduce() {
    static const bool on = [] {
        const bool v = getenv("VDM4CDM_ABLATE_REDUCE") != nullptr;
        if (v) fprintf(stderr, "\n*** libvdm4cdm_hip: VDM4CDM_ABLATE_REDUCE is set - weight-gradient slab reduces are SKIPPED, gradients are WRONG "
                               "(timing ablation only; unset it for any real run) ***\n\n");
        return v;
    }();
    return on;
}

template <typename T, int KS, int STRIDE, int UPS, int TZ, int TY, int NTA = WG<T>::NT, int NTB = WG<T>::NT>
static int launch_wgrad_cfg(WgradArgs w, const WgradPlan& p, float* dw, float* dbias, int accumulate, hipStream_t s) {
    using G = Geo<KS, STRIDE, TZ, TY>;
    ConvArgs& a = w.c;
    if constexpr (UPS != 0) {
        a.Dz /= 2; a.Dy /= 2; a.Dx /= 2;
        a.Iz = a.Sz = a.Dz; a.Iy = a.Sy = a.Dy; a.Ix = a.Sx = a.Dx;
    }
    a.ntz = p.ntz; a.nty = p.nty; a.ntx = p.ntx;
    set_tile_divs(a);
    w.ntiles = p.ntiles; w.P = p.P;
#ifdef VDM_TIMELINE
    a.stamps = g_timeline_stamps;
#endif
    w.bslabs = dbias ? reinterpret_cast<float*>(reinterpret_cast<char*>(w.slabs) + p.slab_bytes) : nullptr;
    const size_t lds = (size_t)((G::HVOX + 15) / 16) * 1024 + (size_t)G::OVOX * 64;
    constexpr bool ROWS = sizeof(T) == 2 && KS == 3 && STRIDE == 1 && UPS == 0 && NTA == 2 && NTB == 2;
    if (p.kernel == VDM_WGRAD_ROWS_ROLL || p.kernel == VDM_WGRAD_ROWS) {
        if constexpr (ROWS) {
            static unsigned long long lds_done_roll = 0, lds_done_rows = 0;
            if (p.kernel == VDM_WGRAD_ROWS_ROLL) {
                a.zsteps = p.zsteps; a.nseg = p.nseg;
                a.fdz = make_fastdiv((uint32_t)a.nseg);
                auto kern = conv_wgrad_rows_kernel<T, TZ, TY, (TZ == 2)>;
                int e = set_lds(kern, lds, lds_done_roll);
                if (e) return e;
                hipLaunchKernelGGL(kern, dim3(p.grid), dim3(256), lds, s, w);
            } else {
                auto kern = conv_wgrad_rows_kernel<T, TZ, TY, false>;
                int e = set_lds(kern, lds, lds_done_rows);
                if (e) return e;
                hipLaunchKernelGGL(kern, dim3(p.grid), dim3(256), lds, s, w);
            }
        }
    } else {
        auto kern = conv_wgrad_kernel<T, KS, STRIDE, UPS, TZ, TY, NTA, NTB>;
        static unsigned long long lds_done = 0;
        int e = set_lds(kern, lds, lds_done);
        if (e) return e;
        hipLaunchKernelGGL(kern, dim3(p.grid), dim3(256), lds, s, w);
    }
    VDM_LAUNCH_CHECK("conv_wgrad_kernel");
    if (ablate_reduce()) return VDM_OK;
    const int total = G::TAPS * a.Cout * a.Cin, nslabs = p.P * p.per_wg;
    if (UPS != 0)
        hipLaunchKernelGGL(wgrad_cls_reduce_kernel, dim3(cdiv(total, 64)), dim3(256), 0, s, (const float*)w.slabs, dw, a.Cout, a.Cin, w.ncb,
                           w.nkb, p.CL, p.P, accumulate);
    else if (!p.grouped)
        hipLaunchKernelGGL(wgrad_reduce_direct_kernel, dim3(cdiv(total, 256)), dim3(256), 0, s,
                           (const float*)w.slabs, dw, G::TAPS, a.Cout, a.Cin, w.ncb, w.nkb, p.CL, nslabs, accumulate);
    else
        hipLaunchKernelGGL(wgrad_reduce_kernel, dim3(cdiv(total, WRED_OUT)), dim3(256), 0, s,
                           (const float*)w.slabs, dw, G::TAPS, a.Cout, a.Cin, w.ncb, w.nkb, p.CL, nslabs, accumulate);
    VDM_LAUNCH_CHECK("wgrad_reduce_kernel");
    if (dbias) {
        hipLaunchKernelGGL(wgrad_bias_reduce_kernel, dim3(cdiv(a.Cout, 16)), dim3(256), 0, s, (const float*)w.bslabs, dbias, a.Cout, p.CL,
                           (UPS != 0 ? 8 : 1) * p.P, accumulate);
        VDM_LAUNCH_CHECK("wgrad_bias_reduce_kernel");
    }
    return VDM_OK;
}

template <typename T>
static int launch_wgrad(const WgradArgs& w, const WgradPlan& p, float* dw, float* db, int acc, hipStream_t s) {
    if (p.kernel == VDM_WGRAD_CLASS) return launch_wgrad_cfg<T, 3, 1, 2, 2, 8>(w, p, dw, db, acc, s);
    if (p.ks == 1) return launch_wgrad_cfg<T, 1, 1, 0, 4, 8>(w, p, dw, db, acc, s);
    if (p.stride == 2) return p.tz == 1 ? launch_wgrad_cfg<T, 3, 2, 0, 1, 4>(w, p, dw, db, acc, s) : launch_wgrad_cfg<T, 3, 2, 0, 2, 4>(w, p, dw, db, acc, s);
    if constexpr (sizeof(T) == 2) {
        if (p.ntb == 1) return launch_wgrad_cfg<T, 3, 1, 0, 2, 8, 2, 1>(w, p, dw, db, acc, s);
        if (p.nta == 1) return launch_wgrad_cfg<T, 3, 1, 0, 2, 8, 1, 2>(w, p, dw, db, acc, s);
    }
    return launch_wgrad_cfg<T, 3, 1, 0, 2, 8>(w, p, dw, db, acc, s);
}

int launch_dgw_reduce(const float* slabs, const float* bslabs, float* dw, float* dbias, int P, int accumulate, hipStream_t s) {
    const int total = 27 * 32 * 32;
    if (ablate_reduce()) return VDM_OK;
    if (P <= 32)
        hipLaunchKernelGGL(wgrad_reduce_direct_kernel, dim3(cdiv(total, 256)), dim3(256), 0, s, slabs, dw, 27, 32, 32, 1, 1, 32, P, accumulate);
    else
        hipLaunchKernelGGL(wgrad_reduce_kernel, dim3(cdiv(total, WRED_OUT)), dim3(256), 0, s, slabs, dw, 27, 32, 32, 1, 1, 32, P, accumulate);
    VDM_LAUNCH_CHECK("wgrad_reduce_kernel(dgw)");
    if (dbias) {
        hipLaunchKernelGGL(wgrad_bias_reduce_kernel, dim3(2), dim3(256), 0, s, bslabs, dbias, 32, 32, P, accumulate);
        VDM_LAUNCH_CHECK("wgrad_bias_reduce_kernel(dgw)");
    }
    return VDM_OK;
}

int launch_wgrad_any(const WgradArgs& w, const WgradPlan& p, float* dw, float* dbias, int accumulate, size_t workspace_bytes, int dtype,
                     hipStream_t s) {
    if (workspace_bytes < p.workspace_bytes) { set_error("conv_wgrad: workspace too small (%zu < %zu)", workspace_bytes, p.workspace_bytes); return VDM_ERR_ARG; }
    if (dbias != nullptr && p.ks == 1) { set_error("conv_wgrad: fused bias gradient is only built for ksize 3"); return VDM_ERR_UNSUPPORTED; }
    if (dtype == VDM_F32) return launch_wgrad<float>(w, p, dw, dbias, accumulate, s);
    return launch_wgrad<bf16_t>(w, p, dw, dbias, accumulate, s);
}

}
```

vdm4cdm_amd/hip_ops.py:

```python
import ctypes as C

import torch

from . import _lib
from ._lib import CondMlp, ConvDesc, GnFold, PACK_DGRAD, PACK_FWD, VDM_BF16, VDM_F32, check

GN_EPS = 1e-5
import os as _os
ABLATE = set(filter(None, _os.environ.get("VDM4CDM_ABLATE", "").split(",")))
if ABLATE or "VDM4CDM_ABLATE_REDUCE" in _os.environ:
    import sys as _sys
    print(f"\n*** vdm4cdm_amd.hip_ops: VDM4CDM_ABLATE={sorted(ABLATE)} / VDM4CDM_ABLATE_REDUCE set - kernels are SKIPPED and results are WRONG "
          "(timing ablations of tools/ablate_step.sh only; Trainer.fit refuses to run) ***\n", file=_sys.stderr, flush=True)


class KernelProfiler:

    def __init__(self, tags=None):
        self.records = []
        self.tags = tags
        self.main_stream = None

    def begin(self):
        e = torch.cuda.Event(enable_timing=True)
        e.record()
        return e

    def end(self, start, key, flops=0.0, nbytes=0.0, exec_flops=None):
        e = torch.cuda.Event(enable_timing=True)
        e.record()
        if self.main_stream is None:
            self.main_stream = torch.cuda.default_stream().cuda_stream
        side = torch.cuda.current_stream().cuda_stream != self.main_stream
        self.records.append((key, start, e, flops, nbytes, flops if exec_flops is None else exec_flops, side))

    def summary(self):
        torch.cuda.synchronize()
        agg = {}
        for key, s, e, fl, nb, xf, side in self.records:
            a = agg.setdefault(key, {"launches": 0, "ms": 0.0, "flops": 0.0, "bytes": 0.0, "exec_flops": 0.0, "side_launches": 0})
            a["launches"] += 1
            a["side_launches"] += 1 if side else 0
            a["ms"] += s.elapsed_time(e)
            a["flops"] += fl
            a["bytes"] += nb
            a["exec_flops"] += xf
        return agg


PROFILER = None
SEED_STEP = None


def _pb(tag="other"):
    if PROFILER is None or (PROFILER.tags is not None and tag not in PROFILER.tags):
        return None
    return PROFILER.begin()


def _pe(ev, key, flops=0.0, nbytes=0.0, exec_flops=None):
    if ev is not None:
        PROFILER.end(ev, key, flops, nbytes, exec_flops)


def _nc_for(cout, dtype=None):
    return 1 if cout <= 16 else (2 if (cout <= 32 or dtype == torch.float32) else 4)


def _tname(dtype):
    return "float" if dtype == torch.float32 else "bf16_t"


def dt_id(dtype):
    if dtype == torch.float32:
        return VDM_F32
    if dtype == torch.bfloat16:
        return VDM_BF16
    raise ValueError(f"unsupported activation dtype {dtype}")


def epl(dtype):
    return 4 if dtype == torch.float32 else 8


def cpad(c, dtype):
    e = epl(dtype)
    return (c + e - 1) // e * e


def _s():
    return torch.cuda.current_stream().cuda_stream


def _scratch(cache, key, numel, dtype, device, floor=0):
    if torch.cuda.is_current_stream_capturing():
        return torch.empty(max(numel, floor), dtype=dtype, device=device)
    ws = cache.get(key)
    if ws is None or ws.numel() < numel:
        ws = cache[key] = torch.empty(max(numel, floor), dtype=dtype, device=device)
    return ws


SIDE_STREAM = None


def _p(t):
    if t is None:
        return None
    assert t.is_cuda, "HIP ops need device tensors"
    if SIDE_STREAM is not None:
        t.record_stream(SIDE_STREAM)
    return t.data_ptr()


def _contig(*ts):
    for t in ts:
        if t is not None:
            assert t.is_contiguous(), "HIP ops need contiguous tensors"


class Conv:

    _ws = {}

    def __init__(self, cin, cout, ksize=3, stride=1, upsample=0, circular=False, out_f32=False):
        self.cin, self.cout, self.ksize, self.stride, self.upsample = cin, cout, ksize, stride, upsample
        self.circular, self.out_f32 = circular, out_f32
        self.wf = self.wd = None
        self._descs = {}

    def desc(self, n, od, oh, ow, dtype, stride=None):
        st = self.stride if stride is None else stride
        key = (n, od, oh, ow, dtype, st)
        d = self._descs.get(key)
        if d is None:
            d = ConvDesc(n=n, od=od, oh=oh, ow=ow, cin=self.cin, cout=self.cout, ksize=self.ksize, stride=st,
                         upsample=self.upsample, pad_mode=1 if self.circular else 0, dtype=dt_id(dtype),
                         out_f32=1 if (self.out_f32 and st == self.stride) else 0)
            self._descs[key] = d
        return d

    def pack(self, w_master, dtype, need_dgrad):
        L = _lib.lib()
        d = self.desc(1, 2, 2, 2, dtype)
        assert w_master.dtype == torch.float32 and w_master.is_contiguous()
        assert w_master.numel() == self.ksize ** 3 * self.cout * self.cin
        self.alloc_packed(w_master.device, dtype, need_dgrad)
        check(L.vdm_conv_pack_weights(d, PACK_FWD, _p(w_master), _p(self.wf), _s()), "vdm_conv_pack_weights(fwd)")
        if need_dgrad:
            check(L.vdm_conv_pack_weights(d, PACK_DGRAD, _p(w_master), _p(self.wd), _s()), "vdm_conv_pack_weights(dgrad)")

    def alloc_packed(self, device, dtype, need_dgrad):
        L = _lib.lib()
        d = self.desc(1, 2, 2, 2, dtype)
        if self.wf is None or self.wf.device != device or self._packed_dtype != dtype:
            self.wf = torch.empty(L.vdm_conv_packed_bytes(d, PACK_FWD), dtype=torch.uint8, device=device)
            self.wd = None
            self._packed_dtype = dtype
        if need_dgrad and self.wd is None:
            self.wd = torch.empty(L.vdm_conv_packed_bytes(d, PACK_DGRAD), dtype=torch.uint8, device=device)

    def _kernel_key(self, d, dgrad, dtype):
        var = _lib.lib().vdm_conv_kernel_variant(d, dgrad)
        t, nc = _tname(dtype), _nc_for(self.cin if dgrad else self.cout, dtype)
        if var == 1:
            return f"conv_cls_kernel<{t},NC{nc},{'B' if dgrad and self.upsample else 'F'}>"
        if var == 2:
            return "conv_kpack_kernel"
        if var == 3:
            return f"conv_fwd_kernel<{t},k3,s1,NC2,split>"
        if var == 4:
            return f"conv_ksplit_kernel<{t},NC4>"
        return f"conv_fwd_kernel<{t},k{self.ksize},s{1 if dgrad else self.stride},NC{nc}>"

    def out_shape(self, x):
        n, d, h, w, _ = x.shape
        if self.stride == 2:
            return (n, d // 2, h // 2, w // 2, self.cout)
        if self.upsample:
            return (n, 2 * d, 2 * h, 2 * w, self.cout)
        return (n, d, h, w, self.cout)

    def gn_in_ok(self, x):
        shp = self.out_shape(x)
        return x.dtype == torch.bfloat16 and bool(_lib.lib().vdm_conv_fwd_gn_supported(self.desc(shp[0], shp[1], shp[2], shp[3], x.dtype)))

    def fwd(self, x, bias=None, nbias=None, residual=None, out=None, gn=False, gn_in=None):
        L = _lib.lib()
        _contig(x, bias, residual)
        assert x.shape[-1] == cpad(self.cin, x.dtype), f"conv input must have {cpad(self.cin, x.dtype)} channels, got {x.shape[-1]}"
        shp = self.out_shape(x)
        if out is None:
            out = torch.empty(shp, dtype=torch.float32 if self.out_f32 else x.dtype, device=x.device)
        assert tuple(out.shape) == shp and out.is_contiguous()
        nstride = 0
        if nbias is not None:
            assert nbias.dtype == torch.float32 and nbias.stride(1) == 1 and nbias.shape[0] == x.shape[0]
            nstride = nbias.stride(0)
        if residual is not None:
            assert residual.shape == out.shape and residual.dtype == x.dtype
        d = self.desc(shp[0], shp[1], shp[2], shp[3], x.dtype)
        part = None
        if gn:
            tiles = L.vdm_conv_gn_tiles(d)
            if tiles > 0:
                part = torch.empty((shp[0], tiles, self.cout, 2), dtype=torch.float32, device=x.device)
        if "conv1" in ABLATE and self.ksize == 1:
            out.gn_partials = None
            return out
        ev = _pb("conv3" if self.ksize == 3 else "other")
        if gn_in is not None:
            G_, st_, gam_, bet_ = gn_in
            _contig(st_, gam_, bet_)
            check(L.vdm_conv_fwd_gn(d, _p(x), _p(self.wf), _p(bias), _p(nbias), nstride, _p(residual), _p(out), _p(part), _p(st_), _p(gam_),
                                    _p(bet_), int(G_), GN_EPS, _s()), "vdm_conv_fwd_gn")
        else:
            check(L.vdm_conv_fwd(d, _p(x), _p(self.wf), _p(bias), _p(nbias), nstride, _p(residual), _p(out), _p(part), _s()), "vdm_conv_fwd")
        out.gn_partials = part
        if ev is not None:
            nvox = shp[0] * shp[1] * shp[2] * shp[3]
            es = x.element_size()
            alg = 2.0 * nvox * self.ksize ** 3 * self.cin * self.cout
            _pe(ev, self._kernel_key(d, 0, x.dtype), alg,
                x.numel() * es + out.numel() * out.element_size() + (residual.numel() * es if residual is not None else 0),
                alg * (8.0 / 27.0) if (self.ksize == 3 and self.upsample) else None)
        return out

    def dgrad(self, dout, residual=None, out=None):
        L = _lib.lib()
        _contig(dout, residual)
        n, od, oh, ow, c = dout.shape
        assert c == cpad(self.cout, dout.dtype)
        if self.stride == 2:
            ishape = (n, 2 * od, 2 * oh, 2 * ow, self.cin)
        elif self.upsample:
            ishape = (n, od // 2, oh // 2, ow // 2, self.cin)
        else:
            ishape = (n, od, oh, ow, self.cin)
        if out is None:
            out = torch.empty(ishape, dtype=dout.dtype, device=dout.device)
        assert tuple(out.shape) == ishape and (residual is None or tuple(residual.shape) == ishape)
        d = self.desc(n, od, oh, ow, dout.dtype)
        if "conv1" in ABLATE and self.ksize == 1:
            return out
        ev = _pb("conv3" if self.ksize == 3 else "other")
        check(L.vdm_conv_dgrad(d, _p(dout), _p(self.wd), _p(residual), _p(out), _s()), "vdm_conv_dgrad")
        if ev is not None:
            nvox = n * od * oh * ow
            es = dout.element_size()
            alg = 2.0 * nvox * self.ksize ** 3 * self.cin * self.cout
            xf = None
            if self.ksize == 3 and self.upsample:
                xf = alg * (8.0 / 27.0)
            elif self.ksize == 3 and self.stride == 2:
                xf = alg
            _pe(ev, self._kernel_key(d, 1, dout.dtype), alg,
                dout.numel() * es + out.numel() * es + (residual.numel() * es if residual is not None else 0), xf)
        return out

    def gn_fold_ok(self, c1, c2, dtype):
        span = 4 * _nc_for(self.cin, dtype)
        return (self.ksize == 3 and self.stride == 1 and not self.upsample and c1 + c2 == self.cin and self.cin % span == 0
                and (c2 == 0 or c1 % span == 0) and self.cin % epl(dtype) == 0)

    def dgrad_gn(self, dout, x1, x2, groups, stats, gamma, beta, keep_mask=None, dropout_p=0.0, out=None):
        L = _lib.lib()
        _contig(dout, x1, x2, stats, gamma, beta, keep_mask)
        n, od, oh, ow, c = dout.shape
        assert c == cpad(self.cout, dout.dtype)
        c1, c2 = x1.shape[-1], (0 if x2 is None else x2.shape[-1])
        assert self.gn_fold_ok(c1, c2, dout.dtype), "dgrad_gn: unsupported channel split"
        assert tuple(x1.shape[:-1]) == (n, od, oh, ow) and x1.dtype == dout.dtype
        if out is None:
            out = torch.empty((n, od, oh, ow, self.cin), dtype=dout.dtype, device=dout.device)
        d = self.desc(n, od, oh, ow, dout.dtype)
        tiles = L.vdm_conv_dgrad_gn_tiles(d)
        part = torch.empty((n, tiles, self.cin, 2), dtype=torch.float32, device=dout.device)
        f = GnFold(x1=_p(x1), x2=_p(x2), c1=c1, c2=c2, groups=groups, stats=_p(stats), gamma=_p(gamma), beta=_p(beta), eps=GN_EPS,
                   inv_keep=1.0 / (1.0 - dropout_p) if keep_mask is not None else 1.0, keep_mask=_p(keep_mask), partials=_p(part))
        ev = _pb("conv3")
        check(L.vdm_conv_dgrad_gn(d, _p(dout), _p(self.wd), _p(out), C.byref(f), _s()), "vdm_conv_dgrad_gn")
        out.gnb_partials = part
        if ev is not None:
            es = dout.element_size()
            _pe(ev, self._kernel_key(d, 1, dout.dtype) + "+gnb", 2.0 * n * od * oh * ow * 27 * self.cin * self.cout,
                dout.numel() * es + 2 * out.numel() * es)
        return out

    def dgw_ok(self, dout, c1, c2):
        n, od, oh, ow, _ = dout.shape
        return (dout.dtype == torch.bfloat16 and self.gn_fold_ok(c1, c2, dout.dtype)
                and bool(_lib.lib().vdm_conv_dgw_supported(self.desc(n, od, oh, ow, dout.dtype))))

    def dgrad_gn_wgrad(self, dout, act, x1, x2, groups, stats, gamma, beta, dw, dbias=None, keep_mask=None, dropout_p=0.0):
        L = _lib.lib()
        _contig(dout, act, x1, x2, stats, gamma, beta, keep_mask, dw, dbias)
        n, od, oh, ow, c = dout.shape
        c1, c2 = x1.shape[-1], (0 if x2 is None else x2.shape[-1])
        assert c == self.cout and act.shape == (n, od, oh, ow, self.cin) and act.dtype == dout.dtype
        d = self.desc(n, od, oh, ow, dout.dtype)
        out = torch.empty((n, od, oh, ow, self.cin), dtype=dout.dtype, device=dout.device)
        part = torch.empty((n, L.vdm_conv_dgw_tiles(d), self.cin, 2), dtype=torch.float32, device=dout.device)
        need = L.vdm_conv_dgw_workspace_bytes(d)
        ws = _scratch(Conv._ws, (dout.device, _s(), "dgw"), need, torch.uint8, dout.device)
        f = GnFold(x1=_p(x1), x2=_p(x2), c1=c1, c2=c2, groups=groups, stats=_p(stats), gamma=_p(gamma), beta=_p(beta), eps=GN_EPS,
                   inv_keep=1.0 / (1.0 - dropout_p) if keep_mask is not None else 1.0, keep_mask=_p(keep_mask), partials=_p(part))
        ev = _pb("conv3")
        check(L.vdm_conv_dgrad_gn_wgrad(d, _p(dout), _p(self.wd), _p(act), _p(out), C.byref(f), _p(dw), _p(dbias), 0, _p(ws), ws.numel(), _s()),
              "vdm_conv_dgrad_gn_wgrad")
        out.gnb_partials = part
        if ev is not None:
            es = dout.element_size()
            _pe(ev, f"conv_dgw_kernel<{_tname(dout.dtype)},k3,s1>(dgrad+gnb+wgrad)", 4.0 * n * od * oh * ow * 27 * self.cin * self.cout,
                (2 * dout.numel() + 3 * out.numel()) * es)
        return out

    def wgrad(self, x, dout, dw, dbias=None, accumulate=False):
        L = _lib.lib()
        _contig(x, dout, dw)
        n, od, oh, ow, c = dout.shape
        assert c == cpad(self.cout, dout.dtype) and x.shape[-1] == cpad(self.cin, x.dtype)
        d = self.desc(n, od, oh, ow, x.dtype)
        need = L.vdm_conv_wgrad_workspace_bytes(d)
        ws = _scratch(Conv._ws, (x.device, _s()), need, torch.uint8, x.device, floor=32 << 20)
        if "wgrad" in ABLATE or ("wgrad1" in ABLATE and self.ksize == 1):
            return dw
        ev = _pb("wgrad" if self.ksize == 3 else "other")
        check(L.vdm_conv_wgrad(d, _p(x), _p(dout), _p(dw), _p(dbias), 1 if accumulate else 0, _p(ws), ws.numel(), _s()), "vdm_conv_wgrad")
        if ev is not None:
            es = x.element_size()
            alg = 2.0 * n * od * oh * ow * self.ksize ** 3 * self.cin * self.cout
            _pe(ev, f"conv_wgrad_kernel<{_tname(x.dtype)},k{self.ksize},s{self.stride},u{self.upsample}>+reduce",
                alg, x.numel() * es + dout.numel() * es, alg * (8.0 / 27.0) if (self.ksize == 3 and self.upsample) else None)
        return dw


def _nv(x):
    n = x.shape[0]
    return n, x.numel() // (n * x.shape[-1])


_gn_ws = {}


def gn_stats(x1, x2, groups, out=None, chsum=False):
    L = _lib.lib()
    _contig(x1, x2)
    n, v = _nv(x1)
    if out is None:
        out = torch.empty((n, groups, 2), dtype=torch.float32, device=x1.device)
    ws = _scratch(_gn_ws, (x1.device, _s()), _lib.GN_STATS_WS_BYTES // 4, torch.float32, x1.device)
    c2 = 0 if x2 is None else x2.shape[-1]
    p1 = getattr(x1, "gn_partials", None)
    p2 = getattr(x2, "gn_partials", None) if x2 is not None else None
    cs = None
    if chsum and p1 is not None and (x2 is None or p2 is not None):
        cs = torch.empty((n, x1.shape[-1] + c2), dtype=torch.float32, device=x1.device)
    ev = _pb()
    check(L.vdm_gn_stats(_p(x1), x1.shape[-1], _p(x2), c2, n, v, groups, dt_id(x1.dtype), _p(out), _p(ws),
                         _p(p1), 0 if p1 is None else p1.shape[1], _p(p2), 0 if p2 is None else p2.shape[1], _p(cs), _s()), "vdm_gn_stats")
    out.chsum = cs
    _pe(ev, "gn_stats", 0.0, (x1.numel() * x1.element_size() if p1 is None else 0)
        + (x2.numel() * x2.element_size() if (x2 is not None and p2 is None) else 0))
    return out


def gn_silu_fwd(x1, x2, groups, stats, gamma, beta, dropout_p=0.0, seed=0, out=None, want_mask=False, linear=False):
    L = _lib.lib()
    _contig(x1, x2, gamma, beta, stats)
    n, v = _nv(x1)
    c1 = x1.shape[-1]
    c2 = 0 if x2 is None else x2.shape[-1]
    if out is None:
        out = torch.empty(x1.shape[:-1] + (c1 + c2,), dtype=x1.dtype, device=x1.device)
    mask = None
    if want_mask and dropout_p > 0.0:
        mask = torch.empty((n, v, (c1 + c2) // epl(x1.dtype)), dtype=torch.uint8, device=x1.device)
    if "gn_fwd" in ABLATE:
        out.keep_mask = mask
        return out
    ev = _pb()
    check(L.vdm_gn_silu_fwd(_p(x1), c1, _p(x2), c2, n, v, groups, dt_id(x1.dtype), _p(stats), _p(gamma), _p(beta), GN_EPS,
                            float(dropout_p), int(seed), _p(out), _p(mask), int(bool(linear)), _p(SEED_STEP), _s()), "vdm_gn_silu_fwd")
    out.keep_mask = mask
    _pe(ev, "gn_silu_fwd", 0.0, 2.0 * out.numel() * out.element_size())
    return out


def gn_skip_supported(c1, c2, cout, dtype):
    if dtype != torch.bfloat16:
        return False, False
    m = _lib.lib().vdm_gn_skip_supported(int(c1), int(c2), int(cout), dt_id(dtype))
    return bool(m & 1), bool(m & 2)


def gn_silu_skip_fwd(x1, x2, groups, stats, gamma, beta, w1, w2, bias):
    L = _lib.lib()
    _contig(x1, x2, gamma, beta, stats, w1, w2, bias)
    n, v = _nv(x1)
    c1 = x1.shape[-1]
    c2 = 0 if x2 is None else x2.shape[-1]
    cout = w1.shape[0]
    y = torch.empty(x1.shape[:-1] + (c1 + c2,), dtype=x1.dtype, device=x1.device)
    sk = torch.empty(x1.shape[:-1] + (cout,), dtype=x1.dtype, device=x1.device)
    y.keep_mask = None
    if "gn_fwd" in ABLATE:
        return y, sk
    ev = _pb()
    check(L.vdm_gn_silu_skip_fwd(_p(x1), c1, _p(x2), c2, n, v, groups, dt_id(x1.dtype), _p(stats), _p(gamma), _p(beta), GN_EPS,
                                 _p(w1), _p(w2), _p(bias), cout, _p(y), _p(sk), _s()), "vdm_gn_silu_skip_fwd")
    _pe(ev, "gn_silu_fwd", 2.0 * n * v * (c1 + c2) * cout, (2.0 * y.numel() + sk.numel()) * y.element_size())
    return y, sk


_skip_ws = {}


def gn_silu_bwd(x1, x2, groups, stats, gamma, beta, dy, dgamma, dbeta, add1=None, add2=None, colsum=None,
                dropout_p=0.0, seed=0, dx1=None, dx2=None, linear=False):
    L = _lib.lib()
    _contig(x1, x2, dy, add1, add2, gamma, beta, dgamma, dbeta, stats)
    n, v = _nv(x1)
    c1 = x1.shape[-1]
    c2 = 0 if x2 is None else x2.shape[-1]
    ev = _pb()
    dyh = dy if (dx1 is not None and dx1.data_ptr() == dy.data_ptr()) else torch.empty_like(dy)
    check(L.vdm_gn_dyh(_p(x1), c1, _p(x2), c2, n, v, groups, dt_id(x1.dtype), _p(stats), _p(gamma), _p(beta), GN_EPS, float(dropout_p),
                       int(seed), _p(dy), _p(dyh), int(bool(linear)), _p(SEED_STEP), _s()), "vdm_gn_dyh")
    dyh.gnb_partials = channel_dot_sums(dyh, x1, x2)
    if colsum is not None and getattr(stats, "chsum", None) is None:
        cs = [channel_dot_sums(t, t)[:, 0, :, 0] for t in (x1, x2) if t is not None]
        stats.chsum = torch.cat(cs, dim=1).contiguous()
    _pe(ev, "gn_dyh+dot_sums", 0.0, 5.0 * dy.numel() * dy.element_size())
    out = gn_bwd_fused(x1, x2, groups, stats, gamma, dyh, dgamma, dbeta, add1=add1, add2=add2, colsum=colsum, dx1=dx1, dx2=dx2)
    if colsum is not None:
        if add1 is not None:
            colsum[:, :c1] += channel_dot_sums(add1, add1)[:, 0, :, 0]
        if add2 is not None:
            colsum[:, c1:c1 + c2] += channel_dot_sums(add2, add2)[:, 0, :, 0]
    return out


def gn_tail_ok(conv_in, x):
    if conv_in.cout != x.shape[-1] or x.shape[0] > 16 or _os.environ.get("VDM4CDM_FUSED_TAIL", "1") == "0":
        return False
    info = _lib.WgradPlanInfo()
    n, od, oh, ow, _ = x.shape
    check(_lib.lib().vdm_conv_wgrad_plan(conv_in.desc(n, od, oh, ow, x.dtype), 1, 0, C.byref(info)), "vdm_conv_wgrad_plan")
    return info.kernel == _lib.WGRAD_THIN_IN


def gn_bwd_fused(x1, x2, groups, stats, gamma, dyh, dgamma, dbeta, add1=None, add2=None, colsum=None, dx1=None, dx2=None, skip=None, tail=None):
    L = _lib.lib()
    _contig(x1, x2, dyh, add1, add2, gamma, dgamma, dbeta, stats)
    n, v = _nv(x1)
    c1 = x1.shape[-1]
    c2 = 0 if x2 is None else x2.shape[-1]
    C_ = c1 + c2
    part = dyh.gnb_partials
    assert part is not None and part.shape[0] == n and part.shape[2] == C_ and dyh.shape[-1] == C_
    red = torch.empty((n, groups, 2), dtype=torch.float32, device=x1.device)
    chan = torch.empty((n, C_, 2), dtype=torch.float32, device=x1.device)
    cstride, chsum = 0, None
    if colsum is not None:
        assert colsum.dtype == torch.float32 and colsum.stride(1) == 1 and colsum.shape[0] == n
        cstride, chsum = colsum.stride(0), getattr(stats, "chsum", None)
        assert chsum is not None, "gn_bwd_fused: colsum needs the per-channel sums (gn_stats(..., chsum=True))"
    if dx1 is None and tail is None:
        dx1 = dyh if x2 is None else torch.empty_like(x1)
    if x2 is not None and dx2 is None:
        dx2 = torch.empty_like(x2)
    ev = _pb()
    check(L.vdm_gn_bwd_finalize(_p(part), part.shape[1], n, C_, groups, v, _p(stats), _p(gamma), GN_EPS, _p(chsum), _p(red), _p(chan),
                                _p(colsum), cstride, _s()), "vdm_gn_bwd_finalize")
    if tail is not None:
        conv_in, xin, dw, dbias = tail
        assert x2 is None and add2 is None and skip is None
        _contig(xin, dw, dbias, add1)
        n_, od, oh, ow, _ = x1.shape
        d = conv_in.desc(n_, od, oh, ow, x1.dtype)
        need = L.vdm_conv_wgrad_workspace_bytes(d)
        ws = _scratch(Conv._ws, (x1.device, _s()), need, torch.uint8, x1.device, floor=32 << 20)
        if "gn_apply" not in ABLATE and "wgrad" not in ABLATE:
            check(L.vdm_gn_bwd_apply_wgrad_thin(_p(x1), c1, n, od, oh, ow, groups, _p(stats), _p(gamma), GN_EPS, _p(dyh), _p(red), _p(chan), _p(add1),
                                                _p(xin), conv_in.cin, 1 if conv_in.circular else 0, _p(dgamma), _p(dbeta), _p(dw), _p(dbias), _p(ws),
                                                ws.numel(), _s()), "vdm_gn_bwd_apply_wgrad_thin")
        _pe(ev, "gn_bwd(finalize+apply)", 2.0 * n * v * 27 * conv_in.cin * c1, (2.0 + (1.0 if add1 is not None else 0.0)) * dyh.numel() * dyh.element_size())
        return None, None
    if skip is not None:
        assert add1 is None and add2 is None
        dout, w1, w2, dw1, dw2 = skip
        _contig(dout, w1, w2, dw1, dw2)
        cout = w1.shape[0]
        nws = L.vdm_gn_skip_ws_floats(c1, c2, cout, n, v)
        ws = _scratch(_skip_ws, (x1.device, _s()), nws, torch.float32, x1.device)
        if "gn_apply" not in ABLATE:
            check(L.vdm_gn_bwd_apply_skip(_p(x1), c1, _p(x2), c2, n, v, groups, dt_id(x1.dtype), _p(stats), _p(gamma), GN_EPS, _p(dyh), _p(red),
                                          _p(chan), _p(dout), _p(w1), _p(w2), cout, _p(dx1), _p(dx2), _p(dgamma), _p(dbeta), _p(dw1), _p(dw2),
                                          _p(ws), ws.numel(), _s()), "vdm_gn_bwd_apply_skip")
        _pe(ev, "gn_bwd(finalize+apply)", 4.0 * n * v * C_ * cout, (3.0 * dyh.numel() + dout.numel()) * dyh.element_size())
        return dx1, dx2
    if "gn_apply" not in ABLATE:
      check(L.vdm_gn_bwd_apply(_p(x1), c1, _p(x2), c2, n, v, groups, dt_id(x1.dtype), _p(stats), _p(gamma), GN_EPS, _p(dyh), _p(red), _p(chan),
                             _p(add1), _p(add2), _p(dx1), _p(dx2), _p(dgamma), _p(dbeta), _s()), "vdm_gn_bwd_apply")
    _pe(ev, "gn_bwd(finalize+apply)", 0.0, (3.0 + (1.0 if add1 is not None else 0.0)) * dyh.numel() * dyh.element_size())
    return dx1, dx2


def pack_input(a, b, dtype, out=None):
    L = _lib.lib()
    _contig(a, b)
    assert a.dtype == torch.float32 and (b is None or (b.dtype == torch.float32 and b.shape == a.shape))
    cp = cpad(2, dtype)
    if out is None:
        out = torch.empty(tuple(a.shape) + (cp,), dtype=dtype, device=a.device)
    check(L.vdm_pack_input(_p(a), _p(b), a.numel(), cp, dt_id(dtype), _p(out), _s()), "vdm_pack_input")
    return out


class CondTable:

    def __init__(self, specs, rows, width):
        self.specs, self.rows, self.width = specs, rows, width
        self.saved = None

    def _descs(self, grads=None):
        arr = (CondMlp * len(self.specs))()
        for k, sp in enumerate(self.specs):
            _contig(sp["input"], sp["w1"], sp["b1"], sp["w2"], sp["b2"], sp["wproj"])
            assert sp["input"].dtype == torch.float32 and sp["input"].shape[0] == self.rows
            d = arr[k]
            d.input, d.in_dim, d.dim, d.sinusoid = _p(sp["input"]), int(sp["in_dim"]), int(sp["w2"].shape[0]), 1 if sp["sinusoid"] else 0
            d.w1, d.b1, d.w2, d.b2, d.wproj = _p(sp["w1"]), _p(sp["b1"]), _p(sp["w2"]), _p(sp["b2"]), _p(sp["wproj"])
            assert tuple(sp["w1"].shape) == (d.dim, d.in_dim) and tuple(sp["wproj"].shape) == (self.width, d.dim)
            if grads is not None:
                g = grads[k]
                _contig(g["w1"], g["b1"], g["w2"], g["b2"], g["wproj"])
                d.dw1, d.db1, d.dw2, d.db2, d.dwproj = _p(g["w1"]), _p(g["b1"]), _p(g["w2"]), _p(g["b2"]), _p(g["wproj"])
        return arr

    def forward(self, save):
        L = _lib.lib()
        dev = self.specs[0]["w1"].device
        arr = self._descs()
        table = torch.empty((self.rows, self.width), dtype=torch.float32, device=dev)
        self.saved = torch.empty(L.vdm_cond_saved_floats(arr, len(self.specs), self.rows), dtype=torch.float32, device=dev) if save else None
        check(L.vdm_cond_table_fwd(arr, len(self.specs), self.rows, self.width, _p(table), _p(self.saved), _s()), "vdm_cond_table_fwd")
        return table

    def backward(self, dtable, grads, dbias=None, dinputs=None):
        L = _lib.lib()
        assert self.saved is not None and dtable.dtype == torch.float32 and dtable.stride(1) == 1 and dtable.shape[0] == self.rows
        arr = self._descs(grads)
        scratch = torch.empty(L.vdm_cond_bwd_scratch_floats(arr, len(self.specs), self.rows, self.width), dtype=torch.float32, device=dtable.device)
        check(L.vdm_cond_table_bwd(arr, len(self.specs), self.rows, self.width, _p(dtable), dtable.stride(0), _p(self.saved), _p(scratch),
                                   _p(dbias), _s()), "vdm_cond_table_bwd")
        if dinputs is not None:
            assert len(dinputs) == len(self.specs)
            for sp, d in zip(self.specs, dinputs):
                assert d is None or (d.dtype == torch.float32 and d.is_contiguous() and tuple(d.shape) == tuple(sp["input"].shape))
            ptrs = (C.c_void_p * len(self.specs))(*[_p(d) for d in dinputs])
            check(L.vdm_cond_input_grad(arr, len(self.specs), self.rows, self.width, _p(self.saved), _p(scratch), ptrs, _s()),
                  "vdm_cond_input_grad")
        self.saved = None


def cond_table_step(table_t, table_v, step_ptr, rows, width, out):
    _contig(table_t, table_v, out)
    check(_lib.lib().vdm_cond_table_step(_p(table_t), _p(table_v), _p(step_ptr), rows, width, _p(out), _s()), "vdm_cond_table_step")
    return out


def augment_batch(fields, consts, samples, crop, out=None):
    L = _lib.lib()
    C_, B = len(fields), len(samples)
    S = fields[0].shape[-1]
    for f in fields:
        assert f.is_cuda and f.dtype == torch.float32 and f.is_contiguous() and f.dim() == 4 and tuple(f.shape[1:]) == (S, S, S), \
            "raw fields must be contiguous fp32 [n_sims, S, S, S] tensors on the GPU"
    nsim = min(f.shape[0] for f in fields)
    if out is None:
        out = [torch.empty(B, 1, crop, crop, crop, device=fields[0].device) for _ in range(C_)]
    ch = (_lib.AugmentChannel * C_)()
    for c, (f, (alpha, mean, std)) in enumerate(zip(fields, consts)):
        _contig(out[c])
        ch[c].field, ch[c].out, ch[c].alpha, ch[c].mean, ch[c].std = f.data_ptr(), out[c].data_ptr(), float(alpha), float(mean), float(std)
    tab = (_lib.AugmentSample * B)()
    for b, (sim, anchor, flip, perm) in enumerate(samples):
        assert 0 <= int(sim) < nsim, f"simulation index {sim} out of range (0..{nsim - 1})"
        tab[b].sim = int(sim)
        for d in range(3):
            tab[b].anchor[d], tab[b].flip[d], tab[b].perm[d] = int(anchor[d]), int(bool(flip[d])), int(perm[d])
    check(L.vdm_augment_batch(ch, C_, int(S), int(crop), tab, B, _s()), "vdm_augment_batch")
    return out


def channel_sums(x, out):
    _contig(x, out)
    c = x.shape[-1]
    check(_lib.lib().vdm_channel_sums(_p(x), x.numel() // c, c, dt_id(x.dtype), _p(out), _s()), "vdm_channel_sums")
    return out


def channel_dot_sums(a, b1, b2=None):
    _contig(a, b1, b2)
    n, c = a.shape[0], a.shape[-1]
    c1 = b1.shape[-1]
    c2 = 0 if b2 is None else b2.shape[-1]
    assert c1 + c2 == c and b1.dtype == a.dtype and b1.shape[:-1] == a.shape[:-1]
    out = torch.empty((n, 1, c, 2), dtype=torch.float32, device=a.device)
    check(_lib.lib().vdm_channel_dot_sums(_p(a), _p(b1), c1, _p(b2), c2, n, a.numel() // (n * c), dt_id(a.dtype), _p(out), _s()),
          "vdm_channel_dot_sums")
    return out


def attn_split_heads(src, sub, nsub, heads, rowmajor=True, transposed=True):
    _contig(src)
    N = src.shape[0]
    C = src.shape[-1] // nsub
    V = src.numel() // (N * nsub * C)
    hd = C // heads
    rm = torch.empty((N, heads, V, hd), dtype=src.dtype, device=src.device) if rowmajor else None
    tr = torch.empty((N, heads, hd, V), dtype=src.dtype, device=src.device) if transposed else None
    check(_lib.lib().vdm_attn_split_heads(_p(src), nsub * C, sub * C, N, V, heads, hd, dt_id(src.dtype), _p(rm), _p(tr), _s()), "vdm_attn_split_heads")
    return rm, tr


def attn_fwd(q, k, vt, scale, out_shape, want_lse=True):
    _contig(q, k, vt)
    N, H, V, hd = q.shape
    out = torch.empty(out_shape, dtype=q.dtype, device=q.device)
# ... 262 lines not shown
```

Measured before the change: 355.1 million voxels/s.

## Add last-block ticket fold for wgrad reduction and merge bias reduce launch

Adds an optional in-kernel fold: each weight-gradient workgroup takes an atomic ticket after writing its partial slab, and the last one per (cout,cin) block pair sums all slabs straight into dw/dbias. This removes the separate reduction kernels and a round trip through the slab workspace. The fold threshold is set to zero, so by default it only runs when forced by a flag. The default path changes too: the weight and bias reductions now run as one merged launch instead of two. The fold path adds atomics, fences and a serialized tail on the last workgroup, and it relies on a persistent ticket buffer that must be reset to zero.

```diff
diff --git a/include/vdm4cdm_hip.h b/include/vdm4cdm_hip.h
--- a/include/vdm4cdm_hip.h
+++ b/include/vdm4cdm_hip.h
@@ -8,7 +8,7 @@
 extern "C" {
 #endif
 
-#define VDM_ABI_VERSION 15
+#define VDM_ABI_VERSION 16
 
 typedef enum { VDM_OK = 0, VDM_ERR_ARG = -1, VDM_ERR_HIP = -2, VDM_ERR_UNSUPPORTED = -3 } vdm_status;
 typedef enum { VDM_F32 = 0, VDM_BF16 = 1 } vdm_dtype;
@@ -87,6 +87,10 @@
 size_t vdm_conv_wgrad_workspace_bytes(const vdm_conv_desc* d);
 int vdm_conv_wgrad(const vdm_conv_desc* d, const void* x, const void* dout, float* dw, float* dbias, int accumulate,
                    void* workspace, size_t workspace_bytes, void* stream);
+#define VDM_WGRAD_SEPARATE_REDUCE 1
+#define VDM_WGRAD_FORCE_FOLD 2
+int vdm_conv_wgrad_fold(const vdm_conv_desc* d, const void* x, const void* dout, float* dw, float* dbias, int accumulate,
+                        void* workspace, size_t workspace_bytes, int32_t* tickets, size_t ticket_bytes, int flags, void* stream);
 
 #define VDM_WGRAD_THIN_IN 0
 #define VDM_WGRAD_THIN_OUT 1
@@ -101,6 +105,10 @@
     int32_t tiles;
     int32_t P;
     size_t workspace_bytes;
+    size_t ticket_bytes;
+    size_t fold_bytes;
+    int32_t fold;
+    int32_t reserved;
 } vdm_wgrad_plan_info;
 int vdm_conv_wgrad_plan(const vdm_conv_desc* d, int want_bias, int accumulate, vdm_wgrad_plan_info* out);
 
diff --git a/vdm4cdm_amd/_lib.py b/vdm4cdm_amd/_lib.py
--- a/vdm4cdm_amd/_lib.py
+++ b/vdm4cdm_amd/_lib.py
@@ -11,6 +11,7 @@
 PAD_ZEROS, PAD_CIRCULAR = 0, 1
 PACK_FWD, PACK_DGRAD = 0, 1
 WGRAD_THIN_IN, WGRAD_THIN_OUT, WGRAD_ROWS, WGRAD_ROWS_ROLL, WGRAD_TAPSPLIT, WGRAD_CLASS = range(6)
+WGRAD_SEPARATE_REDUCE, WGRAD_FORCE_FOLD = 1, 2
 GN_STATS_WS_BYTES = 2048 * 2 * 64 * 4
 
 
@@ -36,7 +37,8 @@
 
 
 class WgradPlanInfo(C.Structure):
-    _fields_ = [(k, C.c_int32) for k in ("kernel", "tz", "ty", "workgroups", "tiles", "P")] + [("workspace_bytes", C.c_size_t)]
+    _fields_ = [(k, C.c_int32) for k in ("kernel", "tz", "ty", "workgroups", "tiles", "P")] + \
+               [("workspace_bytes", C.c_size_t), ("ticket_bytes", C.c_size_t), ("fold_bytes", C.c_size_t), ("fold", C.c_int32), ("reserved", C.c_int32)]
 
 
 class CondMlp(C.Structure):
@@ -62,7 +64,7 @@
 _p, _i, _i64, _u64, _f, _sz = C.c_void_p, C.c_int, C.c_int64, C.c_uint64, C.c_float, C.c_size_t
 _D = C.POINTER(ConvDesc)
 _T = C.POINTER(DdnmTables)
-ABI_VERSION = 15
+ABI_VERSION = 16
 
 SIGNATURES = {
     "vdm_last_error": (C.c_char_p, []),
@@ -86,6 +88,7 @@
     "vdm_conv_dgrad_gn_wgrad": (_i, [_D, _p, _p, _p, _p, C.POINTER(GnFold), _p, _p, _i, _p, _sz, _p]),
     "vdm_conv_wgrad_workspace_bytes": (_sz, [_D]),
     "vdm_conv_wgrad": (_i, [_D, _p, _p, _p, _p, _i, _p, _sz, _p]),
+    "vdm_conv_wgrad_fold": (_i, [_D, _p, _p, _p, _p, _i, _p, _sz, _p, _sz, _i, _p]),
     "vdm_conv_wgrad_plan": (_i, [_D, _i, _i, C.POINTER(WgradPlanInfo)]),
     "vdm_gn_stats": (_i, [_p, _i, _p, _i, _i, _i64, _i, _i, _p, _p, _p, _i, _p, _i, _p, _p]),
     "vdm_gn_silu_fwd": (_i, [_p, _i, _p, _i, _i, _i64, _i, _i, _p, _p, _p, _f, _f, _u64, _p, _p, _i, _p, _p]),
diff --git a/vdm4cdm_amd/csrc/conv_api.hip b/vdm4cdm_amd/csrc/conv_api.hip
--- a/vdm4cdm_amd/csrc/conv_api.hip
+++ b/vdm4cdm_amd/csrc/conv_api.hip
@@ -238,15 +238,22 @@
     out->kernel = p.kernel; out->tz = p.tz; out->ty = p.ty;
     out->workgroups = p.grid; out->tiles = p.ntiles; out->P = p.P;
     out->workspace_bytes = p.workspace_bytes;
+    out->ticket_bytes = p.ticket_bytes; out->fold_bytes = p.fold_bytes; out->fold = p.fold; out->reserved = 0;
     if (want_bias && d->ksize == 1) { set_error("conv_wgrad: fused bias gradient is only built for ksize 3"); return VDM_ERR_UNSUPPORTED; }
     return VDM_OK;
 }
 
 extern "C" int vdm_conv_wgrad(const vdm_conv_desc* d, const void* x, const void* dout, float* dw, float* dbias, int accumulate,
                               void* workspace, size_t workspace_bytes, void* stream) {
+    return vdm_conv_wgrad_fold(d, x, dout, dw, dbias, accumulate, workspace, workspace_bytes, nullptr, 0, 0, stream);
+}
+
+extern "C" int vdm_conv_wgrad_fold(const vdm_conv_desc* d, const void* x, const void* dout, float* dw, float* dbias, int accumulate,
+                                   void* workspace, size_t workspace_bytes, int32_t* tickets, size_t ticket_bytes, int flags, void* stream) {
     int e = validate(d);
     if (e) return e;
     VDM_REQUIRE(x && dout && dw && workspace, "conv_wgrad: NULL pointer");
+    VDM_REQUIRE((flags & ~(VDM_WGRAD_SEPARATE_REDUCE | VDM_WGRAD_FORCE_FOLD)) == 0, "conv_wgrad: unknown flags 0x%x", flags);
     const WgradPlan p = plan_wgrad(d, dbias != nullptr, accumulate != 0);
     hipStream_t s = (hipStream_t)stream;
     if (p.kernel == VDM_WGRAD_THIN_IN || p.kernel == VDM_WGRAD_THIN_OUT) {
@@ -263,7 +270,7 @@
     w.dout = dout; w.dout_stride = cpad(d->cout, d->dtype);
     w.slabs = (float*)workspace;
     w.ncb = p.ncb; w.nkb = p.nkb;
-    return launch_wgrad_any(w, p, dw, dbias, accumulate, workspace_bytes, d->dtype, s);
+    return launch_wgrad_any(w, p, dw, dbias, accumulate, workspace_bytes, d->dtype, tickets, ticket_bytes, flags, s);
 }
 
 
diff --git a/vdm4cdm_amd/csrc/conv_common.h b/vdm4cdm_amd/csrc/conv_common.h
--- a/vdm4cdm_amd/csrc/conv_common.h
+++ b/vdm4cdm_amd/csrc/conv_common.h
@@ -991,6 +991,11 @@
     int P;
     int ntiles;
     int ncb, nkb;
+    int* tickets;
+    float* dw;
+    float* dbias;
+    int fold_grouped;
+    int accumulate;
 };
 
 template <typename T> struct WG;
@@ -1316,6 +1321,8 @@
     int nseg, zsteps;
     int P;
     int per_wg, grouped;
+    int fold;
+    size_t fold_bytes, ticket_bytes;
     int grid;
     size_t slab_bytes;
     size_t workspace_bytes;
@@ -1329,6 +1336,8 @@
 static bool wgrad_roll_enabled() { static const bool on = env_int("VDM4CDM_WGRAD_ROLL", 1) != 0; return on; }
 static int wgrad_s2_tile_z() { static const int v = env_int("VDM4CDM_S2W_TZ", 1); return v == 1 ? 1 : 2; }
 static bool wgrad_grouped_only() { static const bool on = getenv("VDM4CDM_GROUPED_REDUCE") != nullptr; return on; }
+
+constexpr size_t WGRAD_FOLD_MAX_BYTES = 0;
 
 static WgradPlan plan_wgrad_thin(int kernel, int n, int od, int oh, int ow, int cdense) {
     WgradPlan p{};
@@ -1395,6 +1404,9 @@
     p.grouped = p.P * p.per_wg > 32 || wgrad_grouped_only();
     p.slab_bytes = (size_t)p.npairs * p.P * slots * p.CL * p.CL * sizeof(float);
     p.workspace_bytes = p.slab_bytes + (size_t)p.ncb * bias_rows * p.P * p.CL * sizeof(float);
+    p.fold_bytes = p.slab_bytes / ((size_t)p.ncb * p.nkb);
+    p.fold = p.fold_bytes <= WGRAD_FOLD_MAX_BYTES;
+    p.ticket_bytes = (size_t)p.ncb * p.nkb * sizeof(int);
     return p;
 }
 
@@ -1405,7 +1417,7 @@
             hipStream_t s, float* gn_partials = nullptr);
 int launch_dgw_reduce(const float* slabs, const float* bslabs, float* dw, float* dbias, int P, int accumulate, hipStream_t s);
 int launch_wgrad_any(const WgradArgs& w, const WgradPlan& p, float* dw, float* dbias, int accumulate, size_t workspace_bytes, int dtype,
-                     hipStream_t s);
+                     int* tickets, size_t ticket_bytes, int flags, hipStream_t s);
 int launch_wgrad_thin(ThinArgs a, bool gna, const WgradPlan& p, const void* thin_src, int cin, float* dw, float* dbias, void* workspace,
                       size_t workspace_bytes, hipStream_t s);
 
diff --git a/vdm4cdm_amd/csrc/conv_wgrad.hip b/vdm4cdm_amd/csrc/conv_wgrad.hip
--- a/vdm4cdm_amd/csrc/conv_wgrad.hip
+++ b/vdm4cdm_amd/csrc/conv_wgrad.hip
@@ -27,6 +27,98 @@
 #define WG_TL_WRITE(a_) do { } while (0)
 #endif
 
+constexpr int WRED_OUT = 64, WRED_GRP = 4;
+
+__device__ __forceinline__ void f4_add(float4& s, const float4& v) { s.x += v.x; s.y += v.y; s.z += v.z; s.w += v.w; }
+__device__ __forceinline__ void slab_sum4(float4& s, const float* p, size_t stride, int k0, int n, int kstep) {
+    int k = k0;
+    for (; k + 7 * kstep < n; k += 8 * kstep) {
+        float4 v[8];
+#pragma unroll
+        for (int u = 0; u < 8; ++u) v[u] = *reinterpret_cast<const float4*>(p + (size_t)(k + kstep * u) * stride);
+#pragma unroll
+        for (int u = 0; u < 8; ++u) f4_add(s, v[u]);
+    }
+    for (; k < n; k += kstep) f4_add(s, *reinterpret_cast<const float4*>(p + (size_t)k * stride));
+}
+template <int MT, int ST, bool CLS, int CL, int PER_WG>
+__device__ __forceinline__ void wgrad_fold_tail(const WgradArgs& w, int cb, int kb, int* flag) {
+    const int tid = threadIdx.x;
+    asm volatile("s_waitcnt vmcnt(0)" ::: "memory");
+    __syncthreads();
+    if (tid == 0) {
+        __builtin_amdgcn_fence(__ATOMIC_RELEASE, "agent");
+        asm volatile("s_waitcnt vmcnt(0)" ::: "memory");
+        int* cnt = w.tickets + cb * w.nkb + kb;
+        const int last = __hip_atomic_fetch_add(cnt, 1, __ATOMIC_RELAXED, __HIP_MEMORY_SCOPE_AGENT) == (CLS ? 8 : 1) * w.P - 1;
+        if (last) {
+            __hip_atomic_store(cnt, 0, __ATOMIC_RELAXED, __HIP_MEMORY_SCOPE_AGENT);
+            __builtin_amdgcn_fence(__ATOMIC_ACQUIRE, "agent");
+            asm volatile("s_waitcnt vmcnt(0)" ::: "memory");
+        }
+        *flag = last;
+    }
+    __syncthreads();
+    if (*flag == 0) return;
+    const int cout = w.c.Cout, cin = w.c.Cin, acc = w.accumulate;
+    const float* slabs = w.slabs;
+    if (w.bslabs != nullptr && kb == 0 && tid < CL && cb * CL + tid < cout) {
+        const int Pb = (CLS ? 8 : 1) * w.P, co = cb * CL + tid;
+        const float* s = w.bslabs + (size_t)cb * Pb * CL + tid;
+        float tot = 0.f;
+        for (int gp = 0; gp < 16; ++gp) {
+            float sum = 0.f;
+            for (int p = gp; p < Pb; p += 16) sum += s[(size_t)p * CL];
+            tot += sum;
+        }
+        w.dbias[co] = acc ? w.dbias[co] + tot : tot;
+    }
+    constexpr size_t SLAB = (size_t)ST * CL * CL;
+    const int nslabs = w.P * PER_WG;
+    for (int q = tid; q < MT * CL * CL / 4; q += 256) {
+        const int e0 = q * 4, ci_l = e0 % CL, co_l = (e0 / CL) % CL, tap = e0 / (CL * CL);
+        const int co = cb * CL + co_l, ci = kb * CL + ci_l;
+        if (co >= cout || ci >= cin) continue;
+        float4 tot;
+        if constexpr (CLS) {
+            const int tz = tap / 9, ty = (tap / 3) % 3, tx = tap % 3;
+            float4 part[4];
+#pragma unroll
+            for (int sg = 0; sg < 4; ++sg) part[sg] = make_float4(0.f, 0.f, 0.f, 0.f);
+            for (int b = 0; b < 8; ++b) {
+                const int bz = (b >> 2) & 1, by = (b >> 1) & 1, bx = b & 1;
+                const int e = (((tz + 1 - bz) >> 1) << 2) | (((ty + 1 - by) >> 1) << 1) | ((tx + 1 - bx) >> 1);
+                const int pair = (b * w.ncb + cb) * w.nkb + kb;
+                const float* s = slabs + (size_t)pair * w.P * SLAB + ((size_t)e * CL + co_l) * CL + ci_l;
+#pragma unroll
+                for (int sg = 0; sg < 4; ++sg) slab_sum4(part[sg], s, SLAB, sg, w.P, 4);
+            }
+            f4_add(part[0], part[1]);
+            f4_add(part[2], part[3]);
+            tot = part[0];
+            f4_add(tot, part[2]);
+        } else {
+            const float* s = slabs + (size_t)(cb * w.nkb + kb) * nslabs * SLAB + e0;
+            tot = make_float4(0.f, 0.f, 0.f, 0.f);
+            if (w.fold_grouped) {
+#pragma unroll
+                for (int sg = 0; sg < WRED_GRP; ++sg) {
+                    float4 part = make_float4(0.f, 0.f, 0.f, 0.f);
+                    slab_sum4(part, s, SLAB, sg, nslabs, WRED_GRP);
+                    f4_add(tot, part);
+                }
+            } else {
+                slab_sum4(tot, s, SLAB, 0, nslabs, 1);
+            }
+        }
+        float* o = w.dw + ((size_t)tap * cout + co) * cin + ci;
+        const float t4[4] = {tot.x, tot.y, tot.z, tot.w};
+#pragma unroll
+        for (int j = 0; j < 4; ++j)
+            if (ci + j < cin) o[j] = acc ? o[j] + t4[j] : t4[j];
+    }
+}
+
 
 template <typename T, int KS, int STRIDE, int UPS, int TZ, int TY, int NTA = WG<T>::NT, int NTB = WG<T>::NT>
 __global__ void __launch_bounds__(256, 2) conv_wgrad_kernel(const WgradArgs w) {
@@ -190,6 +282,7 @@
     }
     WG_TL(5);
     WG_TL_WRITE(a);
+    if (w.tickets != nullptr) wgrad_fold_tail<G::TAPS, TAPS, CLS, CL, (TAPS > 1) ? 1 : 4>(w, cb, kb, reinterpret_cast<int*>(lds));
 }
 
 template <int V> struct IntC { static constexpr int value = V; };
@@ -357,14 +450,14 @@
         for (int rg = 0; rg < 4; ++rg) slab[(t * CL + ia * 16 + gq * 4 + rg) * CL + jb * 16 + col] = acc[t][rg];
     WG_TL(5);
     WG_TL_WRITE(a);
-}
-
-constexpr int WRED_OUT = 64, WRED_GRP = 4;
-__global__ void __launch_bounds__(256) wgrad_reduce_kernel(const float* __restrict__ slabs, float* __restrict__ dw, int taps,
-                                                          int cout, int cin, int ncb, int nkb, int CL, int nslabs, int accumulate) {
+    if (w.tickets != nullptr) wgrad_fold_tail<27, 27, false, CL, 1>(w, cb, kb, reinterpret_cast<int*>(lds));
+}
+
+__device__ __forceinline__ void wgrad_reduce_block(int block, const float* __restrict__ slabs, float* __restrict__ dw, int taps,
+                                                   int cout, int cin, int ncb, int nkb, int CL, int nslabs, int accumulate) {
     const int total = taps * cout * cin;
     const int o = threadIdx.x % WRED_OUT, sg = threadIdx.x / WRED_OUT;
-    const int i = blockIdx.x * WRED_OUT + o;
+    const int i = block * WRED_OUT + o;
     __shared__ float part[WRED_GRP][WRED_OUT];
     float sum = 0.f;
     if (i < total) {
@@ -391,10 +484,14 @@
         dw[i] = accumulate ? dw[i] + tot : tot;
     }
 }
-__global__ void __launch_bounds__(256) wgrad_reduce_direct_kernel(const float* __restrict__ slabs, float* __restrict__ dw, int taps,
-                                                                 int cout, int cin, int ncb, int nkb, int CL, int nslabs, int accumulate) {
+__global__ void __launch_bounds__(256) wgrad_reduce_kernel(const float* __restrict__ slabs, float* __restrict__ dw, int taps,
+                                                          int cout, int cin, int ncb, int nkb, int CL, int nslabs, int accumulate) {
+    wgrad_reduce_block(blockIdx.x, slabs, dw, taps, cout, cin, ncb, nkb, CL, nslabs, accumulate);
+}
+__device__ __forceinline__ void wgrad_reduce_direct_block(int block, const float* __restrict__ slabs, float* __restrict__ dw, int taps,
+                                                          int cout, int cin, int ncb, int nkb, int CL, int nslabs, int accumulate) {
     const int total = taps * cout * cin;
-    const int i = blockIdx.x * 256 + threadIdx.x;
+    const int i = block * 256 + threadIdx.x;
     if (i >= total) return;
     const int ci = i % cin, co = (i / cin) % cout, tap = i / (cin * cout);
     const int pair = (co / CL) * nkb + ci / CL;
@@ -412,10 +509,14 @@
     for (; k < nslabs; ++k) sum += s[(size_t)k * slab_elems];
     dw[i] = accumulate ? dw[i] + sum : sum;
 }
-__global__ void __launch_bounds__(256) wgrad_bias_reduce_kernel(const float* __restrict__ bslabs, float* __restrict__ dbias, int cout,
-                                                               int CL, int P, int accumulate) {
+__global__ void __launch_bounds__(256) wgrad_reduce_direct_kernel(const float* __restrict__ slabs, float* __restrict__ dw, int taps,
+                                                                 int cout, int cin, int ncb, int nkb, int CL, int nslabs, int accumulate) {
+    wgrad_reduce_direct_block(blockIdx.x, slabs, dw, taps, cout, cin, ncb, nkb, CL, nslabs, accumulate);
+}
+__device__ __forceinline__ void wgrad_bias_reduce_block(int block, const float* __restrict__ bslabs, float* __restrict__ dbias, int cout,
+                                                        int CL, int P, int accumulate) {
     const int c = threadIdx.x & 15, gp = threadIdx.x >> 4;
-    const int co = blockIdx.x * 16 + c;
+    const int co = block * 16 + c;
     __shared__ float part[16][17];
     float sum = 0.f;
     if (co < cout) {
@@ -431,12 +532,16 @@
         dbias[co] = accumulate ? dbias[co] + tot : tot;
     }
 }
-
-__global__ void __launch_bounds__(256) wgrad_cls_reduce_kernel(const float* __restrict__ slabs, float* __restrict__ dw, int cout, int cin,
-                                                              int ncb, int nkb, int CL, int P, int accumulate) {
+__global__ void __launch_bounds__(256) wgrad_bias_reduce_kernel(const float* __restrict__ bslabs, float* __restrict__ dbias, int cout,
+                                                               int CL, int P, int accumulate) {
+    wgrad_bias_reduce_block(blockIdx.x, bslabs, dbias, cout, CL, P, accumulate);
+}
+
+__device__ __forceinline__ void wgrad_cls_reduce_block(int block, const float* __restrict__ slabs, float* __restrict__ dw, int cout, int cin,
+                                                       int ncb, int nkb, int CL, int P, int accumulate) {
     const int total = 27 * cout * cin;
     const int o = threadIdx.x & 63, sg = threadIdx.x >> 6;
-    const int i = blockIdx.x * 64 + o;
+    const int i = block * 64 + o;
     __shared__ float part[4][64];
     float sum = 0.f;
     if (i < total) {
@@ -458,6 +563,21 @@
         dw[i] = accumulate ? dw[i] + tot : tot;
     }
 }
+__global__ void __launch_bounds__(256) wgrad_cls_reduce_kernel(const float* __restrict__ slabs, float* __restrict__ dw, int cout, int cin,
+                                                              int ncb, int nkb, int CL, int P, int accumulate) {
+    wgrad_cls_reduce_block(blockIdx.x, slabs, dw, cout, cin, ncb, nkb, CL, P, accumulate);
+}
+
+template <int MODE>
+__global__ void __launch_bounds__(256) wgrad_reduce_merged_kernel(const float* __restrict__ slabs, float* __restrict__ dw, int taps, int cout,
+                                                                 int cin, int ncb, int nkb, int CL, int nslabs, int accumulate, int dw_blocks,
+                                                                 const float* __restrict__ bslabs, float* __restrict__ dbias, int Pb) {
+    const int b = blockIdx.x;
+    if (b >= dw_blocks) wgrad_bias_reduce_block(b - dw_blocks, bslabs, dbias, cout, CL, Pb, accumulate);
+    else if (MODE == 0) wgrad_reduce_block(b, slabs, dw, taps, cout, cin, ncb, nkb, CL, nslabs, accumulate);
+    else if (MODE == 1) wgrad_reduce_direct_block(b, slabs, dw, taps, cout, cin, ncb, nkb, CL, nslabs, accumulate);
+    else wgrad_cls_reduce_block(b, slabs, dw, cout, cin, ncb, nkb, CL, nslabs, accumulate);
+}
 
 static bool ablate_reduce() {
     static const bool on = [] {
@@ -470,7 +590,7 @@
 }
 
 template <typename T, int KS, int STRIDE, int UPS, int TZ, int TY, int NTA = WG<T>::NT, int NTB = WG<T>::NT>
-static int launch_wgrad_cfg(WgradArgs w, const WgradPlan& p, float* dw, float* dbias, int accumulate, hipStream_t s) {
+static int launch_wgrad_cfg(WgradArgs w, const WgradPlan& p, float* dw, float* dbias, int accumulate, bool legacy, hipStream_t s) {
     using G = Geo<KS, STRIDE, TZ, TY>;
     ConvArgs& a = w.c;
     if constexpr (UPS != 0) {
@@ -484,6 +604,7 @@
     a.stamps = g_timeline_stamps;
 #endif
     w.bslabs = dbias ? reinterpret_cast<float*>(reinterpret_cast<char*>(w.slabs) + p.slab_bytes) : nullptr;
+    w.dw = dw; w.dbias = dbias; w.accumulate = accumulate; w.fold_grouped = p.grouped;
     const size_t lds = (size_t)((G::HVOX + 15) / 16) * 1024 + (size_t)G::OVOX * 64;
     constexpr bool ROWS = sizeof(T) == 2 && KS == 3 && STRIDE == 1 && UPS == 0 && NTA == 2 && NTB == 2;
     if (p.kernel == VDM_WGRAD_ROWS_ROLL || p.kernel == VDM_WGRAD_ROWS) {
@@ -511,8 +632,26 @@
         hipLaunchKernelGGL(kern, dim3(p.grid), dim3(256), lds, s, w);
     }
     VDM_LAUNCH_CHECK("conv_wgrad_kernel");
-    if (ablate_reduce()) return VDM_OK;
-    const int total = G::TAPS * a.Cout * a.Cin, nslabs = p.P * p.per_wg;
+    if (w.tickets != nullptr || ablate_reduce()) return VDM_OK;
+    const int total = G::TAPS * a.Cout * a.Cin, nslabs = p.P * p.per_wg, Pb = (UPS != 0 ? 8 : 1) * p.P;
+    if (!legacy) {
+        const int nb_bias = dbias ? cdiv(a.Cout, 16) : 0;
+        if (UPS != 0) {
+            const int nb = cdiv(total, 64);
+            hipLaunchKernelGGL(wgrad_reduce_merged_kernel<2>, dim3(nb + nb_bias), dim3(256), 0, s, (const float*)w.slabs, dw, G::TAPS, a.Cout,
+                               a.Cin, w.ncb, w.nkb, p.CL, p.P, accumulate, nb, (const float*)w.bslabs, dbias, Pb);
+        } else if (!p.grouped) {
+            const int nb = cdiv(total, 256);
+            hipLaunchKernelGGL(wgrad_reduce_merged_kernel<1>, dim3(nb + nb_bias), dim3(256), 0, s, (const float*)w.slabs, dw, G::TAPS, a.Cout,
+                               a.Cin, w.ncb, w.nkb, p.CL, nslabs, accumulate, nb, (const float*)w.bslabs, dbias, Pb);
+        } else {
+            const int nb = cdiv(total, WRED_OUT);
+            hipLaunchKernelGGL(wgrad_reduce_merged_kernel<0>, dim3(nb + nb_bias), dim3(256), 0, s, (const float*)w.slabs, dw, G::TAPS, a.Cout,
+                               a.Cin, w.ncb, w.nkb, p.CL, nslabs, accumulate, nb, (const float*)w.bslabs, dbias, Pb);
+        }
+        VDM_LAUNCH_CHECK("wgrad_reduce_merged_kernel");
+        return VDM_OK;
+    }
     if (UPS != 0)
         hipLaunchKernelGGL(wgrad_cls_reduce_kernel, dim3(cdiv(total, 64)), dim3(256), 0, s, (const float*)w.slabs, dw, a.Cout, a.Cin, w.ncb,
                            w.nkb, p.CL, p.P, accumulate);
@@ -524,23 +663,23 @@
                            (const float*)w.slabs, dw, G::TAPS, a.Cout, a.Cin, w.ncb, w.nkb, p.CL, nslabs, accumulate);
     VDM_LAUNCH_CHECK("wgrad_reduce_kernel");
     if (dbias) {
-        hipLaunchKernelGGL(wgrad_bias_reduce_kernel, dim3(cdiv(a.Cout, 16)), dim3(256), 0, s, (const float*)w.bslabs, dbias, a.Cout, p.CL,
-                           (UPS != 0 ? 8 : 1) * p.P, accumulate);
+        hipLaunchKernelGGL(wgrad_bias_reduce_kernel, dim3(cdiv(a.Cout, 16)), dim3(256), 0, s, (const float*)w.bslabs, dbias, a.Cout, p.CL, Pb,
+                           accumulate);
         VDM_LAUNCH_CHECK("wgrad_bias_reduce_kernel");
     }
     return VDM_OK;
 }
 
 template <typename T>
-static int launch_wgrad(const WgradArgs& w, const WgradPlan& p, float* dw, float* db, int acc, hipStream_t s) {
-    if (p.kernel == VDM_WGRAD_CLASS) return launch_wgrad_cfg<T, 3, 1, 2, 2, 8>(w, p, dw, db, acc, s);
-    if (p.ks == 1) return launch_wgrad_cfg<T, 1, 1, 0, 4, 8>(w, p, dw, db, acc, s);
-    if (p.stride == 2) return p.tz == 1 ? launch_wgrad_cfg<T, 3, 2, 0, 1, 4>(w, p, dw, db, acc, s) : launch_wgrad_cfg<T, 3, 2, 0, 2, 4>(w, p, dw, db, acc, s);
+static int launch_wgrad(const WgradArgs& w, const WgradPlan& p, float* dw, float* db, int acc, bool legacy, hipStream_t s) {
+    if (p.kernel == VDM_WGRAD_CLASS) return launch_wgrad_cfg<T, 3, 1, 2, 2, 8>(w, p, dw, db, acc, legacy, s);
+    if (p.ks == 1) return launch_wgrad_cfg<T, 1, 1, 0, 4, 8>(w, p, dw, db, acc, legacy, s);
+    if (p.stride == 2) return p.tz == 1 ? launch_wgrad_cfg<T, 3, 2, 0, 1, 4>(w, p, dw, db, acc, legacy, s) : launch_wgrad_cfg<T, 3, 2, 0, 2, 4>(w, p, dw, db, acc, legacy, s);
     if constexpr (sizeof(T) == 2) {
-        if (p.ntb == 1) return launch_wgrad_cfg<T, 3, 1, 0, 2, 8, 2, 1>(w, p, dw, db, acc, s);
-        if (p.nta == 1) return launch_wgrad_cfg<T, 3, 1, 0, 2, 8, 1, 2>(w, p, dw, db, acc, s);
-    }
-    return launch_wgrad_cfg<T, 3, 1, 0, 2, 8>(w, p, dw, db, acc, s);
+        if (p.ntb == 1) return launch_wgrad_cfg<T, 3, 1, 0, 2, 8, 2, 1>(w, p, dw, db, acc, legacy, s);
+        if (p.nta == 1) return launch_wgrad_cfg<T, 3, 1, 0, 2, 8, 1, 2>(w, p, dw, db, acc, legacy, s);
+    }
+    return launch_wgrad_cfg<T, 3, 1, 0, 2, 8>(w, p, dw, db, acc, legacy, s);
 }
 
 int launch_dgw_reduce(const float* slabs, const float* bslabs, float* dw, float* dbias, int P, int accumulate, hipStream_t s) {
@@ -558,12 +697,17 @@
     return VDM_OK;
 }
 
-int launch_wgrad_any(const WgradArgs& w, const WgradPlan& p, float* dw, float* dbias, int accumulate, size_t workspace_bytes, int dtype,
-                     hipStream_t s) {
+int launch_wgrad_any(const WgradArgs& w0, const WgradPlan& p, float* dw, float* dbias, int accumulate, size_t workspace_bytes, int dtype,
+                     int* tickets, size_t ticket_bytes, int flags, hipStream_t s) {
     if (workspace_bytes < p.workspace_bytes) { set_error("conv_wgrad: workspace too small (%zu < %zu)", workspace_bytes, p.workspace_bytes); return VDM_ERR_ARG; }
     if (dbias != nullptr && p.ks == 1) { set_error("conv_wgrad: fused bias gradient is only built for ksize 3"); return VDM_ERR_UNSUPPORTED; }
-    if (dtype == VDM_F32) return launch_wgrad<float>(w, p, dw, dbias, accumulate, s);
-    return launch_wgrad<bf16_t>(w, p, dw, dbias, accumulate, s);
-}
-
-}
+    const bool legacy = (flags & VDM_WGRAD_SEPARATE_REDUCE) != 0;
+    const bool fold = !legacy && tickets != nullptr && !ablate_reduce() && (p.fold || (flags & VDM_WGRAD_FORCE_FOLD) != 0);
+    if (fold && ticket_bytes < p.ticket_bytes) { set_error("conv_wgrad: ticket buffer too small (%zu < %zu)", ticket_bytes, p.ticket_bytes); return VDM_ERR_ARG; }
+    WgradArgs w = w0;
+    w.tickets = fold ? tickets : nullptr;
+    if (dtype == VDM_F32) return launch_wgrad<float>(w, p, dw, dbias, accumulate, legacy, s);
+    return launch_wgrad<bf16_t>(w, p, dw, dbias, accumulate, legacy, s);
+}
+
+}
diff --git a/vdm4cdm_amd/hip_ops.py b/vdm4cdm_amd/hip_ops.py
--- a/vdm4cdm_amd/hip_ops.py
+++ b/vdm4cdm_amd/hip_ops.py
@@ -101,6 +101,20 @@
     return ws
 
 
+_tickets_cache = {}
+TICKET_INTS = 16384
+
+
+def _tickets(device):
+    if torch.cuda.is_current_stream_capturing():
+        return torch.zeros(TICKET_INTS, dtype=torch.int32, device=device)
+    key = (device, _s())
+    t = _tickets_cache.get(key)
+    if t is None:
+        t = _tickets_cache[key] = torch.zeros(TICKET_INTS, dtype=torch.int32, device=device)
+    return t
+
+
 SIDE_STREAM = None
 
 
@@ -124,6 +138,7 @@
     _ws = {}
 
     def __init__(self, cin, cout, ksize=3, stride=1, upsample=0, circular=False, out_f32=False):
+        self._folds = {}
         self.cin, self.cout, self.ksize, self.stride, self.upsample = cin, cout, ksize, stride, upsample
         self.circular, self.out_f32 = circular, out_f32
         self.wf = self.wd = None
@@ -315,7 +330,7 @@
                 (2 * dout.numel() + 3 * out.numel()) * es)
         return out
 
-    def wgrad(self, x, dout, dw, dbias=None, accumulate=False):
+    def wgrad(self, x, dout, dw, dbias=None, accumulate=False, flags=0):
         L = _lib.lib()
         _contig(x, dout, dw)
         n, od, oh, ow, c = dout.shape
@@ -326,7 +341,15 @@
         if "wgrad" in ABLATE or ("wgrad1" in ABLATE and self.ksize == 1):
             return dw
         ev = _pb("wgrad" if self.ksize == 3 else "other")
-        check(L.vdm_conv_wgrad(d, _p(x), _p(dout), _p(dw), _p(dbias), 1 if accumulate else 0, _p(ws), ws.numel(), _s()), "vdm_conv_wgrad")
+        key = (n, od, oh, ow, x.dtype, dbias is not None, bool(accumulate))
+        folds = self._folds.get(key)
+        if folds is None:
+            info = _lib.WgradPlanInfo()
+            check(L.vdm_conv_wgrad_plan(d, int(dbias is not None), int(bool(accumulate)), C.byref(info)), "vdm_conv_wgrad_plan")
+            folds = self._folds[key] = bool(info.fold)
+        tk = _tickets(x.device) if (folds or flags & _lib.WGRAD_FORCE_FOLD) and not flags & _lib.WGRAD_SEPARATE_REDUCE else None
+        check(L.vdm_conv_wgrad_fold(d, _p(x), _p(dout), _p(dw), _p(dbias), 1 if accumulate else 0, _p(ws), ws.numel(), _p(tk),
+                                    0 if tk is None else tk.numel() * 4, flags, _s()), "vdm_conv_wgrad_fold")
         if ev is not None:
             es = x.element_size()
             alg = 2.0 * n * od * oh * ow * self.ksize ** 3 * self.cin * self.cout
```

After: 357.5 million voxels/s (median of 6 runs). Within noise of the previous version (+0.7%).
